# rubendhz/houdini-gsplat-renderer

Hardware: AMD Instinct MI355X
Metric: frames/sec at 1920x1080 + achieved HBM GB/s (blend kernel) (higher is better)
Workload: dtype f32

## Files before the change

houdini-gsplat-renderer_amd/csrc/gsr_api.hip:

```cpp
#include <hip/hip_runtime.h>

#include <cmath>
#include <cstddef>
#include <cstdio>
#include <cstring>
#include <chrono>
#include <algorithm>
#include <new>
#include <type_traits>
#include <vector>

#include "../../include/gsplat_hip.h"
#include "gsr_device.h"
#include "k_binning.h"
#include "k_blend.h"
#include "k_cluster.h"
#include "k_colour.h"
#include "k_preprocess.h"
#ifdef GSR_HOST_TIMING
static double g_t_verdict = 0, g_acc_py = 0, g_acc_pre = 0, g_acc_launch = 0; static long g_acc_n = 0;
static double now_us() { return std::chrono::duration<double, std::micro>(std::chrono::steady_clock::now().time_since_epoch()).count(); }
#endif
#include "k_sort.h"
#include "k_wire.h"
// ... 23 lines not shown
    bool same(const SortKey& o) const
    {
        return gen == o.gen && shard_index == o.shard_index && shard_count == o.shard_count && shard_layout == o.shard_layout && flags == o.flags &&
               band_first == o.band_first && band_tile_rows == o.band_tile_rows &&
               std::memcmp(&cam, &o.cam, sizeof(gsr_camera)) == 0;
    }
};

struct FrameArgs {
    gsr_camera cam{};
    const float* depth = nullptr;
    bool depth_is_device = false;
    float* out = nullptr;
    bool out_is_device = false;
    int aov = 0;
    float* aov_out = nullptr;
    gsr_background bg{};
};

struct FrameJob {
    FrameArgs args;
    bool open = false;
    GsrFrame f{};
    uint32_t n = 0;
    int local_tiles = 0, band_rows = 0, n_super = 0;
    size_t out_px = 0;
    float* target = nullptr;
    int format = 0;
    const float* d_depth = nullptr;
    bool timing = false, timing_all = false, use_map = false;
    bool speculative = false;
    int bn_items = 4;
    uint32_t bn_grid = 0;
    uint32_t k1_grid = 0;
    bool local_sort = false;
    bool sort_failed = false;
    bool redo = false;
    bool ranges_folded = false;
    bool deferred = false;
    bool lazy = false;
    bool cull = false;
    bool direct = false;
    uint32_t ticket = 0;
    int phase = 0;
    bool dcull = false;
    int dpar = 0;
    bool sort_fresh = false;
    bool dblind = false;
    bool dstat = false;
    bool blend_guess_plain = false;
    float2* aov_target = nullptr;
    GsrBgArgs bg{};
};

struct FrameSlot {
    hipStream_t own = nullptr;
    hipStream_t stream = nullptr;
    hipEvent_t ev_done = nullptr;
    hipEvent_t ev_user = nullptr;
    hipEvent_t ev_band[GSR_HOST_BANDS_MAX] = {nullptr, nullptr, nullptr, nullptr, nullptr, nullptr, nullptr, nullptr};
    int bands = 0;
    int band_row[GSR_HOST_BANDS_MAX + 1] = {0, 0, 0, 0, 0, 0, 0, 0, 0};
    hipEvent_t ev_pairs = nullptr;
    GsrRecord* rec = nullptr;
    uint32_t *keyA = nullptr, *keyB = nullptr;
    uint32_t* blk_cnt = nullptr;
    uint2 *valA = nullptr, *valB = nullptr;
    uint32_t* d_n = nullptr;
    float* zwin = nullptr;
    StageBuf depth_stage;
    float* dpyr = nullptr;
    size_t dpyr_cap = 0;
    uint32_t* dactive = nullptr;
    int dpar = 0;
    bool dpyr_built = false;
    bool sorted_dculled = false;
    uint32_t* hist = nullptr;
    size_t hist_cap = 0;
    uint32_t* totals = nullptr;
    uint2* pvA = nullptr;
    size_t pair_cap = 0;
    int32_t *sstart = nullptr, *send = nullptr;
    uint4* tile_work = nullptr;
    size_t tile_cap = 0;
    uint4* tile_work_a = nullptr;
    float* tbuf = nullptr;
    size_t tbuf_cap = 0;
    float* hpyr2 = nullptr;
    uint32_t* slab = nullptr;
    bool slab_dirty = false;
    int32_t* redo = nullptr;
    int32_t* order = nullptr;
    size_t order_cap = 0;
    bool order_valid = false;
    int order_age = 0;
    int order_sig[6] = {0, 0, 0, 0, 0, 0}, order_per_xcd = 0;
    uint32_t* st_scan = nullptr;
    GsrTilePartial* partial = nullptr;
    uint32_t* sup_work = nullptr;
    int sup_par = 0;
    float* hpyr = nullptr;
    float* hpyr_next = nullptr;
    float* hraw = nullptr;
    float* hstat = nullptr;
    bool hstat_valid = false;
    uint32_t* dbg_viol = nullptr;
    int hpyr_re = 0;
    uint32_t* cseg = nullptr;
    uint32_t* ccnt = nullptr;
    uint32_t* d_counts = nullptr;
    uint32_t* bkt_key = nullptr;
    uint2* bkt_val = nullptr;
    uint32_t* bkt_cnt = nullptr;
    GsrSlotHints hints;
    GsrLocalSortPolicy local_pol;
    unsigned long long* h_end = nullptr;
    unsigned long long* h_rows = nullptr;
    unsigned long long* h_rows_dev = nullptr;
    uint32_t rows_ticket = 0;
    int rows_tiles_y = 0;
    unsigned long long* h_end_dev = nullptr;
    bool horizon_valid = false;
    int horizon_sig[7] = {0, 0, 0, 0, 0, 0, 0};
    gsr_camera horizon_cam{};
    bool sorted_culled = false;
    unsigned long long* lazy_ctr = nullptr;
    uint32_t* colour_evals = nullptr;
    bool last_lazy = false;
    StageBuf fb;
    StageBuf aovb;
    float* fb32 = nullptr;
    size_t fb32_cap = 0;
    StageBuf bgb;
    unsigned long long* counters = nullptr;
    unsigned long long* h_total = nullptr;
    unsigned long long* h_total_dev = nullptr;
    uint32_t ticket = 0;
    unsigned long long* h_counters = nullptr;
    unsigned long long* d_frame = nullptr;
    bool sort_valid = false;
    SortKey sort_key{};
    uint32_t key_min = 0;
    FrameJob job;
    int last_tiles_x = 0, last_local_ty = 0, last_supers = 0;
    uint32_t last_cc_groups = 0, last_cc_per = 0;
    uint32_t last_pairs = 0;
    int super_tile = 0, stiles_x = 0, stiles_y = 0;
    uint64_t frame_id = 0;
    hipEvent_t ev[GSR_STAGE_EVENTS];
    bool ev_pending = false;
    bool ev_all = false;
    bool ev_ok = false;
};

struct gsr_context {
    int device = 0;
    hipStream_t own_stream = nullptr;
    hipStream_t stream = nullptr;

    uint32_t n = 0, cap = 0;
    bool has_sh = false;
    float origin[3] = {0, 0, 0};
    uint64_t geo_gen = 0;
    bool has_geometry = false;
    float4* geoA = nullptr;
    uint4* geoB = nullptr;
    uint4* col = nullptr;
    uint4* colrow = nullptr;
    int col_chunks = 0;
    float4* geoA2 = nullptr;
    uint4 *geoB2 = nullptr, *col2 = nullptr, *colrow2 = nullptr;
    float4 *clusA2 = nullptr, *clusB2 = nullptr;
    uint32_t* perm = nullptr;
    std::vector<int32_t> h_perm;
    float4 *clusA = nullptr, *clusB = nullptr;
    uint32_t nclus = 0;
    uint32_t* prefix = nullptr;
    uint32_t* prefix_all = nullptr;
    uint32_t* prefix_none = nullptr;
    bool prefix_valid = false;
    bool uploading = false;
    uint32_t up_total = 0, up_filled = 0;
    bool bbox_ok = false;
    double bb_lo[3] = {0, 0, 0}, bb_hi[3] = {0, 0, 0};

    FrameSlot slot[GSR_MAX_SLOTS];
    uint32_t* pos_order = nullptr;
    size_t pos_cap = 0;
    bool pos_valid = false;
    uint64_t pos_gen = 0;
    float pos_cam[3] = {0, 0, 0}, last_cam[3] = {0, 0, 0};
    uint32_t pos_kmin = 0, pos_kmax = 0;
    bool last_cam_set = false;
    uint32_t* blk_pre = nullptr;
    size_t blk_pre_cap = 0;
    int opt_order_keep = 32;
    int opt_fuse_order = 1;
    int opt_mid_sort = 1;
    int opt_host_bands = 4;
    hipStream_t copy_stream = nullptr;
    int opt_k1_scatter = 1;
    int opt_scatter_direct = 1;
    int opt_bn_items = 0;
    int nslots = 1;

    int32_t* tile_map = nullptr;
    size_t map_cap = 0;
    int map_w = 0, map_h = 0, map_si = -1, map_sc = 0, map_rpb = -1, map_first = -1, map_shift = -1, map_grid = 0;

    int shard_index = 0, shard_count = 1, shard_layout = 0;
    int band_first = 0, band_tile_rows = -1;
    int opt_row_work = 0;
    int target_format = GSR_TARGET_RGBA32F;
    int opt_swizzle = 2, opt_timing = 1, opt_sort_cache = 1, opt_super = 0, opt_flags = 0, opt_deferred = 0, opt_lazy = 1, opt_cull = 1, opt_timing_every = 1;
    int opt_cluster = 1, opt_morton = 1, opt_local_sort = 1;
    int opt_slab = 1;
    int slab_frac = 40, slab_min = 4096, slab_max = 8192;
    bool classic_once = false;

    gsr_stats st{};
    uint64_t frame_no = 0;
    size_t pair_want = 0;
    int64_t lazy_base = 0;
    uint32_t* lazy_hint = nullptr;
    bool lazy_pays = false;
    GsrCullPolicy cull_pol;
    GsrSlabPolicy slab_pol;
    bool prefix_cheaper = false;
    bool depth_active = false;
    bool order_pays = false;
    unsigned long long* wire_zbuf = nullptr;
    float* wire_out = nullptr;
    uint32_t* wire_inv = nullptr;
    uint64_t wire_inv_gen = 0;
    size_t wire_cap = 0;
    char* stage = nullptr;
    size_t stage_cap = 0;
    char* stage_raw = nullptr;
    size_t stage_raw_cap = 0;
    uint32_t *up_kA = nullptr, *up_kB = nullptr, *up_vA = nullptr, *up_vB = nullptr;
    size_t up_sort_cap = 0;
    float* up_part = nullptr;
    hipEvent_t up_ev[4] = {nullptr, nullptr, nullptr, nullptr};
    double up_t_begin = 0.0, up_h2d_ms = 0.0, up_quant_ms = 0.0;
    bool vis_on = false;
    GsrVisRule vis{};
    float* alpha0 = nullptr;
    uint32_t* vis_mask = nullptr;
    unsigned long long* vis_counters = nullptr;
    unsigned long long* vis_h_counters = nullptr;
    int64_t vis_hidden = 0;
    float* alpha0_2 = nullptr;
    uint32_t* rm_h_total = nullptr;
    int64_t rm_calls = 0, rm_last = 0;
    double rm_ms[4] = {0.0, 0.0, 0.0, 0.0};
    int64_t add_calls = 0, add_last = 0, add_grows = 0;
    double add_ms[4] = {0.0, 0.0, 0.0, 0.0};
    int64_t rd_calls = 0, rd_last = 0;
    double rd_ms[4] = {0.0, 0.0, 0.0, 0.0};
};

static inline uint32_t div_up(uint32_t a, uint32_t b) { return (a + b - 1) / b; }

#ifdef GSR_KPROF
extern "C" int gsr_debug_kprof_blocks(unsigned int* out8192) {
    hipDeviceSynchronize();
    return hipMemcpyFromSymbol(out8192, HIP_SYMBOL(g_kprof_blk), sizeof(g_kprof_blk)) == hipSuccess ? 0 : -1;
}
extern "C" int gsr_debug_kprof(unsigned long long* out128) {
    hipDeviceSynchronize();
    return hipMemcpyFromSymbol(out128, HIP_SYMBOL(g_kprof), sizeof(g_kprof)) == hipSuccess ? 0 : -1;
}
#endif
#ifdef SW_PROFILE
extern "C" int gsr_debug_sw_profile(unsigned long long* out8) {
    hipDeviceSynchronize();
    hipMemcpyFromSymbol(out8, HIP_SYMBOL(g_sw_prof), 64);
    return 0;
}
// ... 50 lines not shown
    ok = ok && hipEventCreateWithFlags(&sl.ev_pairs, hipEventDisableTiming) == hipSuccess;
    ok = ok && hipMalloc(reinterpret_cast<void**>(&sl.counters), 8 * sizeof(unsigned long long)) == hipSuccess;
    ok = ok && hipMalloc(reinterpret_cast<void**>(&sl.d_n), sizeof(uint32_t)) == hipSuccess;
    ok = ok && hipMemset(sl.d_n, 0, sizeof(uint32_t)) == hipSuccess;
    ok = ok && hipMalloc(reinterpret_cast<void**>(&sl.totals), 512 * sizeof(uint32_t)) == hipSuccess;
    ok = ok && hipMalloc(reinterpret_cast<void**>(&sl.lazy_ctr), 2 * sizeof(unsigned long long)) == hipSuccess;
    ok = ok && hipMemset(sl.lazy_ctr, 0, 2 * sizeof(unsigned long long)) == hipSuccess;
    ok = ok && hipMalloc(reinterpret_cast<void**>(&sl.colour_evals), 256 * sizeof(uint32_t)) == hipSuccess;
    ok = ok && hipMemset(sl.colour_evals, 0, 256 * sizeof(uint32_t)) == hipSuccess;
    ok = ok && hipMalloc(reinterpret_cast<void**>(&sl.hpyr), GSR_PYR_FLOATS * sizeof(float)) == hipSuccess;
    ok = ok && hipMalloc(reinterpret_cast<void**>(&sl.hpyr_next), GSR_PYR_FLOATS * sizeof(float)) == hipSuccess;
    ok = ok && hipMalloc(reinterpret_cast<void**>(&sl.hraw), (size_t)GSR_MAX_TILES_SIDE * GSR_MAX_TILES_SIDE * sizeof(float)) == hipSuccess;
    ok = ok && hipMalloc(reinterpret_cast<void**>(&sl.hstat), (size_t)GSR_MAX_TILES_SIDE * GSR_MAX_TILES_SIDE * sizeof(float)) == hipSuccess;
    ok = ok && hipMalloc(reinterpret_cast<void**>(&sl.hpyr2), GSR_PYR_FLOATS * sizeof(float)) == hipSuccess;
    ok = ok && hipMalloc(reinterpret_cast<void**>(&sl.slab), (GSR_SLAB_BINS + 8) * sizeof(uint32_t)) == hipSuccess;
    ok = ok && hipMemset(sl.slab, 0, (GSR_SLAB_BINS + 8) * sizeof(uint32_t)) == hipSuccess;
    ok = ok && hipMalloc(reinterpret_cast<void**>(&sl.ccnt), CC_MAX_GROUPS * sizeof(uint32_t)) == hipSuccess;
    ok = ok && hipMalloc(reinterpret_cast<void**>(&sl.bkt_key), (size_t)BK_BUCKETS * BK_CAP * sizeof(uint32_t)) == hipSuccess;
    ok = ok && hipMalloc(reinterpret_cast<void**>(&sl.bkt_val), (size_t)BK_BUCKETS * BK_CAP * sizeof(uint2)) == hipSuccess;
    ok = ok && hipMalloc(reinterpret_cast<void**>(&sl.bkt_cnt), (size_t)BK_BUCKETS * BK_STRIDE * sizeof(uint32_t)) == hipSuccess;
    ok = ok && hipMemset(sl.bkt_cnt, 0, (size_t)BK_BUCKETS * BK_STRIDE * sizeof(uint32_t)) == hipSuccess;
    ok = ok && hipMalloc(reinterpret_cast<void**>(&sl.d_counts), 4 * sizeof(uint32_t)) == hipSuccess;
    ok = ok && hipMemset(sl.d_counts, 0, 4 * sizeof(uint32_t)) == hipSuccess;
    ok = ok && hipHostMalloc(reinterpret_cast<void**>(&sl.h_end), sizeof(unsigned long long), hipHostMallocMapped | hipHostMallocCoherent) == hipSuccess;
    if (ok) sl.h_end[0] = 0ull;
    ok = ok && hipHostGetDevicePointer(reinterpret_cast<void**>(&sl.h_end_dev), sl.h_end, 0) == hipSuccess;
    ok = ok && hipMalloc(reinterpret_cast<void**>(&sl.st_scan), 512 * sizeof(uint32_t)) == hipSuccess;
    ok = ok && hipMemset(sl.st_scan, 0, 512 * sizeof(uint32_t)) == hipSuccess;
    ok = ok && hipMalloc(reinterpret_cast<void**>(&sl.partial), (size_t)(GSR_MAX_TILES_SIDE / 8) * (GSR_MAX_TILES_SIDE / 8) * sizeof(GsrTilePartial)) == hipSuccess;
    ok = ok && hipMalloc(reinterpret_cast<void**>(&sl.sup_work), 512 * sizeof(uint32_t)) == hipSuccess;
    ok = ok && hipMemset(sl.sup_work, 0, 512 * sizeof(uint32_t)) == hipSuccess;
    ok = ok && hipHostMalloc(reinterpret_cast<void**>(&sl.h_total), 4 * sizeof(unsigned long long), hipHostMallocMapped | hipHostMallocCoherent) == hipSuccess;
    if (ok) { sl.h_total[0] = 0ull; sl.h_total[1] = 0ull; sl.h_total[2] = 0ull; sl.h_total[3] = 0ull; }
    ok = ok && hipHostGetDevicePointer(reinterpret_cast<void**>(&sl.h_total_dev), sl.h_total, 0) == hipSuccess;
    ok = ok && hipHostMalloc(reinterpret_cast<void**>(&sl.h_counters), 8 * sizeof(unsigned long long), 0) == hipSuccess;
    if (ok) for (int j = 0; j < 8; ++j) sl.h_counters[j] = 0;
    ok = ok && hipMalloc(reinterpret_cast<void**>(&sl.d_frame), 8 * sizeof(unsigned long long)) == hipSuccess;
    ok = ok && hipMemset(sl.d_frame, 0, 8 * sizeof(unsigned long long)) == hipSuccess;
    ok = ok && hipMemset(sl.counters, 0, 8 * sizeof(unsigned long long)) == hipSuccess;
    if (ok) {
        for (int k = 0; k < GSR_STAGE_EVENTS; ++k) sl.ev[k] = nullptr;
        sl.ev_ok = true;
        for (int k = 0; k < GSR_STAGE_EVENTS && ok; ++k) ok = hipEventCreate(&sl.ev[k]) == hipSuccess;
    }
    return ok;
}

static void slot_free_splat_arrays(FrameSlot& sl)
{
    dev_free(sl.rec); dev_free(sl.keyA); dev_free(sl.keyB); dev_free(sl.valA); dev_free(sl.valB); dev_free(sl.blk_cnt);
    dev_free(sl.zwin); dev_free(sl.cseg);
    sl.sort_valid = false;
}

struct SlotSplatArrays {
    GsrRecord* rec = nullptr;
    uint32_t *keyA = nullptr, *keyB = nullptr, *blk_cnt = nullptr, *cseg = nullptr;
    uint2 *valA = nullptr, *valB = nullptr;
    float* zwin = nullptr;
    void release() { dev_free(rec); dev_free(keyA); dev_free(keyB); dev_free(valA); dev_free(valB); dev_free(blk_cnt); dev_free(zwin); dev_free(cseg); }
};
static int alloc_splat_arrays(SlotSplatArrays& a, size_t cap)
{
    int rc = GSR_OK;
    if ((rc = dev_alloc(&a.rec, cap)) || (rc = dev_alloc(&a.keyA, cap + 256)) || (rc = dev_alloc(&a.keyB, cap + 256)) ||
        (rc = dev_alloc(&a.valA, cap + 256)) || (rc = dev_alloc(&a.valB, cap + 256)) ||
        (rc = dev_alloc(&a.zwin, cap)) || (rc = dev_alloc(&a.blk_cnt, cap / 256 + 16)) ||
        (rc = dev_alloc(&a.cseg, cap / GSR_CLUSTER + (size_t)CC_THREADS * 64 + 16)))
        a.release();
    return rc;
}
static void slot_take_splat_arrays(FrameSlot& sl, SlotSplatArrays& a)
{
    slot_free_splat_arrays(sl);
    sl.rec = a.rec; sl.keyA = a.keyA; sl.keyB = a.keyB; sl.valA = a.valA; sl.valB = a.valB; sl.blk_cnt = a.blk_cnt; sl.zwin = a.zwin; sl.cseg = a.cseg;
    a = SlotSplatArrays{};
}

static void slot_destroy(FrameSlot& sl)
{
    slot_free_splat_arrays(sl);
    dev_free(sl.hist); dev_free(sl.totals);
    dev_free(sl.pvA);
    dev_free(sl.sstart); dev_free(sl.send); dev_free(sl.tile_work); dev_free(sl.order); dev_free(sl.sup_work); sl.fb.release(); dev_free(sl.fb32); sl.aovb.release(); sl.bgb.release();
    dev_free(sl.hpyr); dev_free(sl.hpyr_next); dev_free(sl.hraw); dev_free(sl.hstat); dev_free(sl.hpyr2); dev_free(sl.slab); dev_free(sl.tile_work_a); dev_free(sl.tbuf); dev_free(sl.ccnt); dev_free(sl.bkt_key); dev_free(sl.bkt_val); dev_free(sl.bkt_cnt); dev_free(sl.d_counts); dev_free(sl.st_scan); dev_free(sl.partial);
    if (sl.h_end) (void)hipHostFree(sl.h_end); if (sl.h_rows) (void)hipHostFree(sl.h_rows); sl.depth_stage.release(); dev_free(sl.dpyr); dev_free(sl.dactive);
    dev_free(sl.redo); dev_free(sl.lazy_ctr); dev_free(sl.colour_evals);
    dev_free(sl.counters); dev_free(sl.d_n);
    if (sl.h_total) (void)hipHostFree(sl.h_total);
    if (sl.h_counters) (void)hipHostFree(sl.h_counters);
    dev_free(sl.d_frame);
    if (sl.ev_ok)
        for (int k = 0; k < GSR_STAGE_EVENTS; ++k)
            if (sl.ev[k]) (void)hipEventDestroy(sl.ev[k]);
    if (sl.ev_done) (void)hipEventDestroy(sl.ev_done);
    if (sl.ev_user) (void)hipEventDestroy(sl.ev_user);
    for (int k = 0; k < GSR_HOST_BANDS_MAX; ++k) if (sl.ev_band[k]) (void)hipEventDestroy(sl.ev_band[k]);
    if (sl.ev_pairs) (void)hipEventDestroy(sl.ev_pairs);
    if (sl.own) (void)hipStreamDestroy(sl.own);
}

extern "C" int gsr_create(int device, gsr_context** out)
{
    if (!out) return set_err(GSR_E_INVALID, "gsr_create: out is NULL");
    *out = nullptr;
    int ndev = gsr_device_count();
    if (ndev <= 0) return set_err(GSR_E_NO_DEVICE, "gsr_create: no HIP device visible");
    if (device < 0 || device >= ndev) return set_err(GSR_E_NO_DEVICE, "gsr_create: device %d out of range (0..%d)", device, ndev - 1);
    HIP_TRY(hipSetDevice(device));
    gsr_context* c = new (std::nothrow) gsr_context();
    if (!c) return set_err(GSR_E_OOM, "gsr_create: host allocation failed");
    c->device = device;
    if (const char* e = std::getenv("GSR_ORDER_KEEP")) c->opt_order_keep = std::atoi(e);
    if (const char* e = std::getenv("GSR_SCATTER_DIRECT")) c->opt_scatter_direct = std::atoi(e);
    if (const char* e = std::getenv("GSR_K1_SCATTER")) c->opt_k1_scatter = std::atoi(e);
    if (const char* e = std::getenv("GSR_HOST_BANDS")) c->opt_host_bands = std::min(std::max(std::atoi(e), 1), GSR_HOST_BANDS_MAX);
    if (const char* e = std::getenv("GSR_MID_SORT")) c->opt_mid_sort = std::atoi(e);
    if (const char* e = std::getenv("GSR_FUSE_ORDER")) c->opt_fuse_order = std::atoi(e);
    if (const char* e = std::getenv("GSR_SLAB_FRAC")) { const int v = std::atoi(e); if (v >= 1 && v <= 255) c->slab_frac = v; }
    if (const char* e = std::getenv("GSR_SLAB_MIN")) { const int v = std::atoi(e); if (v >= 1) c->slab_min = v; }
    if (const char* e = std::getenv("GSR_SLAB_MAX")) { const int v = std::atoi(e); if (v >= 1) c->slab_max = v; }
    if (const char* e = std::getenv("GSR_BN_ITEMS")) { const int v = std::atoi(e); if (v == 1 || v == 2 || v == 4) c->opt_bn_items = v; }
    hipError_t e = hipStreamCreateWithFlags(&c->own_stream, hipStreamNonBlocking);
    if (e != hipSuccess) { delete c; return set_err(GSR_E_HIP, "hipStreamCreate failed: %s", hipGetErrorString(e)); }
    c->stream = c->own_stream;
    bool ok = true;
    for (int k = 0; k < GSR_MAX_SLOTS && ok; ++k) ok = slot_init(c->slot[k]);
    if (!ok) {
        gsr_destroy(c);
        return set_err(GSR_E_HIP, "gsr_create: allocating frame slots (streams/events/mailboxes) failed");
    }
    if (hipMalloc(reinterpret_cast<void**>(&c->prefix), 256 * 4) != hipSuccess ||
        hipMalloc(reinterpret_cast<void**>(&c->prefix_all), 256 * 4) != hipSuccess ||
        hipMalloc(reinterpret_cast<void**>(&c->prefix_none), 256 * 4) != hipSuccess ||
        hipMemset(c->prefix, 0xff, 256 * 4) != hipSuccess || hipMemset(c->prefix_all, 0xff, 256 * 4) != hipSuccess ||
        hipMemset(c->prefix_none, 0, 256 * 4) != hipSuccess ||
        hipMalloc(reinterpret_cast<void**>(&c->lazy_hint), 4) != hipSuccess || hipMemset(c->lazy_hint, 0, 4) != hipSuccess) {
        gsr_destroy(c);
        return set_err(GSR_E_HIP, "gsr_create: allocating the colour-prefix tables failed");
    }
    c->st.record_bytes = (int32_t)sizeof(GsrRecord);
    c->st.pair_bytes = 8;
    *out = c;
    return GSR_OK;
}

static void vis_drop_mask(gsr_context* c)
{
    dev_free(c->vis_mask);
    if (c->vis.n_volumes == 0) { c->vis_on = false; c->vis_hidden = 0; }
}

static void free_geometry(gsr_context* c)
{
    dev_free(c->geoA); dev_free(c->geoB); dev_free(c->col); dev_free(c->colrow);
    dev_free(c->perm); dev_free(c->clusA); dev_free(c->clusB); c->nclus = 0; c->h_perm.clear();
    dev_free(c->geoA2); dev_free(c->geoB2); dev_free(c->col2); dev_free(c->colrow2); dev_free(c->clusA2); dev_free(c->clusB2);
    dev_free(c->alpha0);
    dev_free(c->alpha0_2);
    vis_drop_mask(c);
    for (int k = 0; k < GSR_MAX_SLOTS; ++k) slot_free_splat_arrays(c->slot[k]);
    c->cap = 0; c->n = 0;
}

extern "C" void gsr_destroy(gsr_context* c)
{
    if (!c) return;
    (void)hipSetDevice(c->device);
    (void)sync_all(c);
    gsr_internal_comm_release(c);
    free_geometry(c);
    for (int k = 0; k < GSR_MAX_SLOTS; ++k) slot_destroy(c->slot[k]);
    dev_free(c->tile_map);
    dev_free(c->wire_zbuf); dev_free(c->wire_out); dev_free(c->wire_inv); dev_free(c->stage); dev_free(c->stage_raw);
    dev_free(c->up_kA); dev_free(c->up_kB); dev_free(c->up_vA); dev_free(c->up_vB); dev_free(c->up_part);
    for (int k = 0; k < 4; ++k) if (c->up_ev[k]) (void)hipEventDestroy(c->up_ev[k]);
    dev_free(c->prefix); dev_free(c->prefix_all); dev_free(c->prefix_none); dev_free(c->lazy_hint);
    dev_free(c->pos_order); dev_free(c->blk_pre); dev_free(c->vis_counters);
    if (c->vis_h_counters) (void)hipHostFree(c->vis_h_counters);
    if (c->rm_h_total) (void)hipHostFree(c->rm_h_total);
    if (c->own_stream) (void)hipStreamDestroy(c->own_stream);
    if (c->copy_stream) (void)hipStreamDestroy(c->copy_stream);
    delete c;
}

extern "C" int gsr_set_stream(gsr_context* c, void* s)
{
    if (!c) return set_err(GSR_E_INVALID, "gsr_set_stream: ctx is NULL");
    if (gsr_internal_comm_set_user_stream(c, s, c->own_stream)) return GSR_OK;
    HIP_TRY(hipSetDevice(c->device));
    int rc = sync_all(c);
    if (rc) return rc;
    c->stream = s ? reinterpret_cast<hipStream_t>(s) : c->own_stream;
    for (int k = 0; k < GSR_MAX_SLOTS; ++k) c->slot[k].stream = c->slot[k].own;
    return GSR_OK;
}

extern "C" int gsr_set_option(gsr_context* c, int option, int value)
{
    if (!c) return set_err(GSR_E_INVALID, "gsr_set_option: ctx is NULL");
    switch (option) {
// ... 849 lines not shown
    c->st.ms_tile_sort = ms[3] + ms[4];
    c->st.ms_blend = ms[5];
    float tot = 0.0f;
    (void)hipEventElapsedTime(&tot, e[0], e[6]);
    c->st.ms_total = tot;
    c->st.blend_ms_total += ms[5];
    c->st.blend_launches += 1;
    c->st.frame_ms_total += tot;
    c->st.stage_ms_total[0] += ms[0];
    c->st.stage_ms_total[1] += ms[1];
    c->st.stage_ms_total[2] += ms[2];
    c->st.stage_ms_total[3] += ms[3] + ms[4];
    c->st.stage_ms_total[4] += ms[5];
    c->st.stage_frames += 1;
}

static inline int mark(FrameSlot& sl, int k)
{
    const FrameJob& j = sl.job;
    if (j.timing && (j.timing_all || k >= 5)) HIP_TRY(hipEventRecord(sl.ev[k], sl.stream));
    return GSR_OK;
}

static GsrRangeArgs range_args(gsr_context* c, FrameSlot& sl)
{
    const FrameJob& j = sl.job;
    GsrRangeArgs a;
    a.totals = sl.totals; a.n_super = j.n_super; a.sstart = sl.sstart; a.send = sl.send; a.host_total = sl.h_total_dev;
    a.ticket = j.ticket; a.max_pairs = (unsigned long long)GSR_MAX_PAIRS; a.redo_count = reinterpret_cast<uint32_t*>(sl.lazy_ctr);
    a.lazy_hint = c->lazy_hint; a.n_sorted = sl.d_n; a.k1_counts = sl.d_counts; a.sorted_keys = sl.keyA;
    a.depth_active = j.dcull ? sl.dactive + j.dpar : (const uint32_t*)nullptr;
    return a;
}

static inline void tile_sig(const GsrFrame& f, int* sig )
{
    const int now[6] = {f.width, f.height, f.shard_rpb > 0 ? f.shard_first : f.shard_index, f.shard_count, f.shard_rpb, f.super_shift};
    std::memcpy(sig, now, sizeof now);
}

static inline int32_t list_cap(const FrameSlot& sl) { return (int32_t)std::min<size_t>(sl.pair_cap, (size_t)0x7fffffff); }

static GsrSumArgs sum_args(const FrameJob& j)
{
    GsrSumArgs g;
    g.n_tiles = j.local_tiles; g.tiles_x = j.f.tiles_x; g.tiles_y = j.f.tiles_y; g.shard = gsr_frame_shard(j.f, 0);
    g.super_shift = j.f.super_shift; g.stiles_x = j.f.stiles_x; g.n_super = j.n_super;
    return g;
}

static GsrHorizonArgs horizon_args(const gsr_context* c, const FrameSlot& sl)
{
    const GsrFrame& f = sl.job.f;
    GsrHorizonArgs hz{};
    hz.list_cap = list_cap(sl); hz.lists = sl.pvA; hz.geoA = c->geoA; hz.idx_mask = f.idx_mask;
    for (int l = 0; l < GSR_PYR_LEVELS; ++l) hz.pyr_off[l] = f.pyr_off[l];
    hz.cam[0] = f.cam[0]; hz.cam[1] = f.cam[1]; hz.cam[2] = f.cam[2];
    return hz;
}

static int queue_blend(gsr_context* c, FrameSlot& sl, bool with_depth, bool guarded)
{
    const FrameJob& j = sl.job;
    const GsrFrame& f = j.f;
    hipStream_t s = sl.stream;
    if (j.local_tiles <= 0) return GSR_OK;
    if (!j.direct) HIP_TRY(hipStreamWaitEvent(s, sl.ev_user, 0));
    GsrBlendArgs a;
    a.guard = guarded ? sl.dactive + j.dpar : (const uint32_t*)nullptr; a.guard_want = 0u;
    {
        const bool persp = f.pr[8] == 0.0f && f.pr[9] == 0.0f && f.pr[12] == 0.0f && f.pr[13] == 0.0f && f.pr[14] == -1.0f && f.pr[15] == 0.0f;
        a.near_alpha = persp ? 0.5f * (1.0f - f.pr[10]) : 0.0f;
        a.near_scale = persp ? 1.12f : 0.0f;
    }
    a.tile_cov = (with_depth && j.dcull && !j.dblind) ? sl.dpyr + 4 * sl.dpyr_cap : (const float*)nullptr;
    a.idx_mask = f.idx_mask; a.zq0 = f.zq0; a.zqs = f.zqs;
    a.tile_dmax = (with_depth && j.dcull && !j.dblind && f.idx_mask != 0xffffffffu) ? sl.dpyr + (size_t)(2 * j.dpar) * sl.dpyr_cap + f.pyr_off[0] : (const float*)nullptr;
    a.width = f.width; a.height = f.height; a.tiles_x = f.tiles_x; a.local_tiles = j.local_tiles;
    a.shard = gsr_frame_shard(f, 0); a.band_rows = j.band_rows;
    a.super_shift = f.super_shift; a.rect_shift = f.rect_shift; a.stiles_x = f.stiles_x; a.use_map = j.use_map ? 1 : 0; a.flags = f.flags;
    a.list_cap = list_cap(sl);
    a.sup_work = (a.use_map && c->opt_swizzle >= 2 && sl.sup_work) ? sl.sup_work + 256 * sl.sup_par : nullptr;
    a.slab = j.phase; a.tbuf = sl.tbuf; a.tile_work_a = sl.tile_work_a;
    uint4* const tw = j.phase == 1 ? sl.tile_work_a : sl.tile_work;
    int sig[6];
    tile_sig(f, sig);
    const bool ordered = a.use_map && c->opt_swizzle >= 2 && sl.order_valid && std::memcmp(sig, sl.order_sig, sizeof sig) == 0;
    const int32_t* tmap = ordered ? sl.order : c->tile_map;
    const unsigned grid = ordered ? (unsigned)(8 * sl.order_per_xcd) : a.use_map ? (unsigned)c->map_grid : (unsigned)j.local_tiles;
    GsrLazyArgs lz;
    lz.f = f; lz.colrow = c->colrow;
    lz.redo = j.lazy ? sl.redo : nullptr;
    lz.redo_count = reinterpret_cast<uint32_t*>(sl.lazy_ctr);
    const bool over = j.bg.kind != 0;
    a.out_format = j.format; a.out_packed = (j.format != GSR_TARGET_RGBA32F || over) ? (void*)j.target : nullptr;
    float4* tgt = reinterpret_cast<float4*>((j.format != GSR_TARGET_RGBA32F || over) ? sl.fb32 : j.target);
    auto launch = [&](auto kernel, unsigned g, const int32_t* map, uint4* work, auto... tail) {
        hipLaunchKernelGGL(kernel, dim3(g), dim3(256), 0, s, a, map, sl.pvA, sl.sstart, sl.send, sl.rec, tgt, work, sl.zwin, j.d_depth, lz, tail...);
    };
    auto launch_verb = [&](auto plain, auto aov, auto bg, unsigned g, const int32_t* map, uint4* work) {
        if (j.aov_target) launch(aov, g, map, work, j.aov_target);
        else if (over) launch(bg, g, map, work, j.bg);
        else launch(plain, g, map, work);
    };
    int nb = 1;
    if (!j.args.out_is_device && j.phase != 1 && c->opt_host_bands > 1 && c->shard_count == 1 && c->band_tile_rows < 0 && f.local_tiles_y >= 4 * c->opt_host_bands) nb = c->opt_host_bands;
    if (nb > 1 && !c->copy_stream && hipStreamCreateWithFlags(&c->copy_stream, hipStreamNonBlocking) != hipSuccess) { c->copy_stream = nullptr; nb = 1; (void)hipGetLastError(); }
    for (int b = 0; b < nb && nb > 1; ++b)
        if (!sl.ev_band[b] && hipEventCreateWithFlags(&sl.ev_band[b], hipEventDisableTiming) != hipSuccess) { sl.ev_band[b] = nullptr; nb = 1; (void)hipGetLastError(); }
    sl.bands = nb;
    for (int b = 0; b < nb; ++b) {
        a.row_lo = nb > 1 ? (int)((int64_t)f.local_tiles_y * b / nb) : 0;
        a.row_hi = nb > 1 ? (int)((int64_t)f.local_tiles_y * (b + 1) / nb) : 0x7fffffff;
        sl.band_row[b] = a.row_lo; sl.band_row[b + 1] = nb > 1 ? a.row_hi : f.local_tiles_y;
        if (with_depth) launch_verb(k_blend<true>, k_blend_aov<true>, k_blend_over<true>, grid, tmap, tw);
        else launch_verb(k_blend<false>, k_blend_aov<false>, k_blend_over<false>, grid, tmap, tw);
        if (j.lazy && with_depth) launch_verb(k_blend_lazy<true>, k_blend_aov_lazy<true>, k_blend_over_lazy<true>, (unsigned)j.local_tiles, c->tile_map, sl.tile_work);
        else if (j.lazy) launch_verb(k_blend_lazy<false>, k_blend_aov_lazy<false>, k_blend_over_lazy<false>, (unsigned)j.local_tiles, c->tile_map, sl.tile_work);
        if (nb > 1) HIP_TRY(hipEventRecord(sl.ev_band[b], s));
    }
    HIP_TRY(hipGetLastError());
    return GSR_OK;
}

static int queue_back_end(gsr_context* c, FrameSlot& sl)
{
    const FrameJob& j = sl.job;
    const GsrFrame& f = j.f;
    hipStream_t s = sl.stream;
    int rc;
    if ((rc = mark(sl, 3))) return rc;
    if (j.n > 0) {
        const uint32_t nblk = div_up(j.n, (uint32_t)BN_THREADS * (uint32_t)j.bn_items);
        const size_t lds = (size_t)4 * j.bn_items * j.n_super * (8 + 4);
        const GsrShard shd = gsr_frame_shard(f, f.rect_shift);
        const GsrRangeArgs ra = j.ranges_folded ? range_args(c, sl) : GsrRangeArgs{};
        const uint32_t bn_extra = (uint32_t)BN_SPLIT_TILES * (uint32_t)std::max(f.stiles_y - 1, 0);
        const uint32_t grid = std::min(nblk, j.bn_grid) + bn_extra + (j.ranges_folded ? 1u : 0u);
#define GSR_PLACE(I) hipLaunchKernelGGL((f.idx_mask != 0xffffffffu ? k_bin_place<I, true> : k_bin_place<I, false>), dim3(grid), dim3(BN_THREADS), lds, s, sl.valA, sl.d_n,          \
                                        f.super_shift - f.rect_shift, shd, f.stiles_x, j.n_super, sl.hist, sl.sstart, nblk, (uint32_t)sl.pair_cap, sl.pvA, ra,   \
                                        f.idx_mask != 0xffffffffu ? sl.zwin : (const float*)nullptr, f.zq0, f.zqs)
        if (j.bn_items == 1) GSR_PLACE(1); else if (j.bn_items == 2) GSR_PLACE(2); else GSR_PLACE(4);
#undef GSR_PLACE
        HIP_TRY(hipGetLastError());
    }
    if ((rc = mark(sl, 4))) return rc;
    if (j.lazy && j.n > 0) {
        const bool predict = c->prefix_valid && !(f.flags & GSR_FLAG_LAZY_NO_PREFIX);
        hipLaunchKernelGGL(k_colour_prefix, dim3((unsigned)(j.n_super * CL_BLOCKS_PER_LIST)), dim3(CL_THREADS), 0, s, f, sl.pvA,
                           sl.sstart, sl.send, (f.flags & GSR_FLAG_LAZY_NO_PREFIX) ? c->prefix_none : (predict ? c->prefix : c->prefix_all),
                           (int)list_cap(sl), c->colrow, sl.rec, sl.colour_evals);
        HIP_TRY(hipGetLastError());
    }
    if ((rc = mark(sl, 5))) return rc;
    sl.job.blend_guess_plain = j.d_depth != nullptr && j.dcull && !c->depth_active && !j.deferred && j.f.idx_mask == 0xffffffffu && !j.aov_target && j.bg.kind == 0;
    if ((rc = queue_blend(c, sl, j.d_depth != nullptr && !sl.job.blend_guess_plain, sl.job.blend_guess_plain))) return rc;
    return mark(sl, 6);
}

static int queue_frame_end(gsr_context* c, FrameSlot& sl)
{
    const FrameJob& j = sl.job;
    hipStream_t s = sl.stream;
    const GsrSumArgs g = sum_args(j);
    GsrHorizonArgs hz{};
    hz.list_cap = list_cap(sl);
    if (c->opt_cull && c->opt_cull != 3 && j.n > 0 && !j.deferred && (c->opt_cull >= 2 || j.cull || j.phase == 2 || (c->cull_pol.vis_unculled >= 300000u && c->cull_pol.holdoff <= 2))) {
        hz = horizon_args(c, sl);
        hz.raw = sl.hraw; hz.pyr_in = sl.hpyr; hz.pyr_out = sl.hpyr_next; hz.dilate = j.f.cull_dilate; hz.culled = j.cull ? 1 : 0;
        hz.host_end = j.cull ? sl.h_end_dev : nullptr; hz.ticket = j.ticket;
        hz.stat = sl.hstat;
        hz.stat_in_use = (j.cull && j.dcull && j.dstat) ? 1 : 0;
        hz.depth_culled = (j.dcull && !j.dblind) ? 1 : 0;
        static const bool dbgv = std::getenv("GSR_DEBUG_VIOL") != nullptr;
        if (dbgv) {
            if (!sl.dbg_viol && hipMalloc(reinterpret_cast<void**>(&sl.dbg_viol), 80 * 4) != hipSuccess) sl.dbg_viol = nullptr;
            if (sl.dbg_viol) (void)hipMemsetAsync(sl.dbg_viol, 0, 80 * 4, s);
            hz.dbg = sl.dbg_viol;
        }
    }
    if (j.phase == 2) { hz.slab = 2; hz.tile_work_a = sl.tile_work_a; }
    const int nblocks8 = ((j.f.tiles_x + 7) >> 3) * ((j.f.tiles_y + 7) >> 3);
    hipLaunchKernelGGL(k_tile_pass, dim3((unsigned)nblocks8), dim3(64), 0, s, sl.tile_work, g, sl.sstart, sl.send, hz, sl.partial, sl.st_scan);
    uint32_t* const prefix_arg = (j.f.sh_order > 0 && c->opt_lazy) ? c->prefix : (uint32_t*)nullptr;
    const uint32_t* const redo_arg = j.lazy ? reinterpret_cast<const uint32_t*>(sl.lazy_ctr) : (const uint32_t*)nullptr;
    uint32_t* const work_next = sl.sup_work ? sl.sup_work + 256 * (sl.sup_par ^ 1) : (uint32_t*)nullptr;
    sl.horizon_valid = hz.raw != nullptr;
    sl.hstat_valid = hz.raw != nullptr;
    int osig[6];
    tile_sig(j.f, osig);
    const bool order_due = c->opt_swizzle >= 3 || (c->opt_swizzle == 2 && c->order_pays);
    const bool order_kept = !order_due && c->opt_swizzle == 2 && c->opt_order_keep > 0 && sl.order_valid && sl.order_age < c->opt_order_keep &&
                            std::memcmp(osig, sl.order_sig, sizeof osig) == 0;
    const bool order_refresh = !order_due && !order_kept && c->opt_swizzle == 2 && c->opt_order_keep > 0 && c->n >= 1000000u;
    if (order_kept) sl.order_age += 1; else sl.order_valid = false;
    const bool order_now = j.use_map && (order_due || order_refresh) && j.local_tiles > 0 && j.n_super <= 256 && sl.sup_work;
    const int per_xcd = 2 * ((j.n_super + 15) / 16) << (2 * j.f.super_shift);
    if (order_now && (size_t)8 * per_xcd > sl.order_cap) {
        const int rc = regrow(s, sl.order, sl.order_cap, (size_t)8 * per_xcd, (size_t)8 * per_xcd);
        if (rc) return rc;
    }
    const bool fused_order = order_now && c->opt_fuse_order != 0;
    if (sl.horizon_valid) sl.hpyr_re = std::min(c->cull_pol.dilate, GSR_DILATE_EXACT_MAX);
    if (fused_order) {
        const GsrOrderArgs oa{sl.tile_work, j.f.tiles_y, sl.sup_work + 256 * sl.sup_par, per_xcd, sl.order};
        const int ndil = sl.horizon_valid ? nblocks8 : 0;
        hipLaunchKernelGGL(k_frame_end_order, dim3(9u + (unsigned)((ndil + TO_THREADS / 64 - 1) / (TO_THREADS / 64))), dim3(TO_THREADS), 0, s, sl.partial, nblocks8, ndil, g, sl.counters, sl.d_n, sl.d_frame,
                           prefix_arg, redo_arg, sl.colour_evals, sl.lazy_ctr + 1, sl.sstart, sl.send, c->lazy_hint, work_next, hz, sl.st_scan, sl.hpyr_re, oa);
        HIP_TRY(hipGetLastError());
    } else if (sl.horizon_valid) {
        hipLaunchKernelGGL(k_frame_end, dim3((unsigned)nblocks8 + 1u), dim3(SW_THREADS), 0, s, sl.partial, nblocks8, g, sl.counters, sl.d_n, sl.d_frame,
                           prefix_arg, redo_arg, sl.colour_evals, sl.lazy_ctr + 1, sl.sstart, sl.send, c->lazy_hint, work_next, hz, sl.st_scan, sl.hpyr_re);
        HIP_TRY(hipGetLastError());
    } else {
        hipLaunchKernelGGL(k_sum_work, dim3(1), dim3(SW_THREADS), 0, s, sl.partial, nblocks8, g, sl.counters, sl.d_n, sl.d_frame,
                           prefix_arg, redo_arg, sl.colour_evals, sl.lazy_ctr + 1, sl.sstart, sl.send, c->lazy_hint, work_next, hz, sl.st_scan);
        HIP_TRY(hipGetLastError());
    }
    if (sl.horizon_valid) {
        std::swap(sl.hpyr, sl.hpyr_next);
        tile_sig(j.f, sl.horizon_sig);
        sl.horizon_sig[6] = (int)c->geo_gen;
        sl.horizon_cam = j.args.cam;
    }
    if (order_now) {
        if (!fused_order) {
            hipLaunchKernelGGL(k_tile_order, dim3(8), dim3(TO_THREADS), 0, s, sl.tile_work, g, j.f.tiles_y, sl.sup_work + 256 * sl.sup_par,
                               per_xcd, sl.order);
            HIP_TRY(hipGetLastError());
        }
        std::memcpy(sl.order_sig, osig, sizeof osig);
        sl.order_per_xcd = per_xcd;
        sl.order_valid = true;
        sl.order_age = 0;
    }
    if (c->opt_row_work && sl.h_rows_dev) {
        hipLaunchKernelGGL(k_row_work, dim3((unsigned)((j.f.tiles_y + RW_THREADS / 64 - 1) / (RW_THREADS / 64))), dim3(RW_THREADS), 0, s, sl.tile_work,
                           j.phase == 2 ? sl.tile_work_a : (const uint4*)nullptr, g, sl.h_rows_dev, j.ticket);
        HIP_TRY(hipGetLastError());
        sl.rows_ticket = j.ticket; sl.rows_tiles_y = j.f.tiles_y;
    }
    sl.sup_par ^= 1;
    if (j.f.sh_order > 0 && c->opt_lazy) c->prefix_valid = j.phase == 0;
    sl.last_lazy = j.lazy;
    if (j.timing) { sl.ev_pending = true; sl.ev_all = j.timing_all; }
    if (!j.args.out_is_device) {
        const size_t bpp = (size_t)gsr_format_pixel_bytes(j.format);
        if (sl.bands > 1 && c->copy_stream) {
            for (int b = 0; b < sl.bands; ++b) {
                const size_t r0 = std::min<size_t>((size_t)sl.band_row[b] * GSR_TILE, (size_t)j.band_rows), r1 = std::min<size_t>((size_t)sl.band_row[b + 1] * GSR_TILE, (size_t)j.band_rows);
                if (r1 <= r0) continue;
                const size_t off = r0 * (size_t)j.f.width * bpp;
                HIP_TRY(hipStreamWaitEvent(c->copy_stream, sl.ev_band[b], 0));
                HIP_TRY(hipMemcpyAsync(reinterpret_cast<char*>(j.args.out) + off, static_cast<const char*>(sl.fb.p) + off, (r1 - r0) * (size_t)j.f.width * bpp, hipMemcpyDeviceToHost, c->copy_stream));
            }
            HIP_TRY(hipStreamSynchronize(c->copy_stream));
        } else {
            HIP_TRY(hipMemcpyAsync(j.args.out, sl.fb.p, j.out_px * bpp, hipMemcpyDeviceToHost, s));
        }
        if (j.aov_target) HIP_TRY(hipMemcpyAsync(j.args.aov_out, sl.aovb.p, j.out_px * 8, hipMemcpyDeviceToHost, s));
        HIP_TRY(hipStreamSynchronize(s));
    }
    if (!j.direct) {
        HIP_TRY(hipEventRecord(sl.ev_done, s));
        HIP_TRY(hipStreamWaitEvent(c->stream, sl.ev_done, 0));
    }
    return GSR_OK;
}

static int queue_slab_mid(gsr_context* c, FrameSlot& sl)
{
    const FrameJob& j = sl.job;
    hipStream_t s = sl.stream;
    const GsrSumArgs g = sum_args(j);
    GsrHorizonArgs hz = horizon_args(c, sl);
    hz.raw = (c->opt_cull && c->opt_cull != 3) ? sl.hraw : nullptr;
    const int nblocks8 = ((j.f.tiles_x + 7) >> 3) * ((j.f.tiles_y + 7) >> 3);
    hipLaunchKernelGGL(k_slab_mid, dim3((unsigned)nblocks8), dim3(64), 0, s, sl.tile_work_a, g, sl.sstart, sl.send, hz, sl.hpyr2,
                       sl.slab + GSR_SLAB_BINS, j.f.key_min);
    HIP_TRY(hipGetLastError());
    return GSR_OK;
}

static int frame_abort(FrameSlot& sl, int rc)
{
    sl.job.open = false;
    if (sl.stream) (void)hipStreamSynchronize(sl.stream);
    return rc;
}

static int wait_mailbox(FrameSlot& sl, volatile unsigned long long* box, uint32_t ticket, const char* what, unsigned long long* out)
{
    unsigned long long v = *box;
    if ((uint32_t)(v >> 32) != ticket) {
        const auto t0 = std::chrono::steady_clock::now();
        for (unsigned long spins = 1; (uint32_t)(v >> 32) != ticket; ++spins) {
            if ((spins & 0xffu) == 0 && std::chrono::steady_clock::now() - t0 > std::chrono::microseconds(GSR_SPIN_US)) {
                const hipError_t q = hipStreamSynchronize(sl.stream);
                if (q != hipSuccess) return set_err(GSR_E_HIP, "gsr_render: waiting for the %s: %s", what, hipGetErrorString(q));
                v = *box;
                if ((uint32_t)(v >> 32) != ticket) return set_err(GSR_E_HIP, "gsr_render: the frame finished without delivering its %s", what);
                break;
            }
            __builtin_ia32_pause();
            v = *box;
        }
    }
    *out = v;
    return GSR_OK;
}

static bool camera_jumped(const gsr_context* c, const gsr_camera& was, const gsr_camera& now)
{
    if (!c->bbox_ok) return false;
    double diag2 = 0.0;
    for (int k = 0; k < 3; ++k) diag2 += ((double)c->bb_hi[k] - c->bb_lo[k]) * ((double)c->bb_hi[k] - c->bb_lo[k]);
    if (!(diag2 > 0.0) || !std::isfinite(diag2)) return false;
// ... 198 lines not shown
    if (!c->has_geometry) return set_err(GSR_E_NO_GEOMETRY, "gsr_render: nothing uploaded");
    HIP_TRY(hipSetDevice(c->device));

    FrameSlot& sl = c->slot[c->frame_no % (uint64_t)c->nslots];
    slot = &sl;
    int rc = frame_finish(c, sl);
    if (rc) return rc;
    hipStream_t want = (c->nslots == 1) ? c->stream : sl.own;
    if (want != sl.stream) {
        HIP_TRY(hipStreamSynchronize(sl.stream));
        sl.stream = want;
    }
    if (sl.pair_cap > 0 && sl.pair_cap < c->pair_want && (rc = regrow(sl.stream, sl.pvA, sl.pair_cap, c->pair_want + 4, c->pair_want))) return rc;

    FrameJob& j = sl.job;
    j = FrameJob();
    j.args = a;
    build_frame(c, cam, &j.f);
    j.n = c->n;
    j.local_tiles = j.f.tiles_x * j.f.local_tiles_y;
    j.band_rows = ctx_band_rows(c, cam->height);
    j.out_px = (size_t)j.band_rows * cam->width;
    j.n_super = j.f.stiles_x * j.f.stiles_y;
    j.use_map = c->opt_swizzle != 0;
    return GSR_OK;
}

static void plan_frame(gsr_context* c, FrameSlot& sl, FrontEnd& fe, bool allow_cull, int phase_in)
{
    FrameJob& j = sl.job;
    const FrameArgs& a = j.args;
    const gsr_camera* cam = &a.cam;
    const GsrFrame& f = j.f;
    fe.key_now = SortKey{c->geo_gen, c->shard_index, c->shard_count, c->shard_layout, c->opt_flags, c->band_first, c->band_tile_rows, *cam};
    int sig[7] = {0, 0, 0, 0, 0, 0, (int)c->geo_gen};
    tile_sig(f, sig);
    GsrPlanIn in;
    in.phase_in = phase_in; in.allow_cull = allow_cull; in.out_is_device = a.out_is_device; in.has_depth = a.depth != nullptr;
    in.n = j.n; in.nclus = c->nclus; in.sh_order = f.sh_order; in.key_min = f.key_min; in.key_max = f.key_max;
    in.opt_deferred = c->opt_deferred; in.opt_lazy = c->opt_lazy; in.opt_cull = c->opt_cull; in.opt_slab = c->opt_slab; in.opt_cluster = c->opt_cluster;
    in.opt_sort_cache = c->opt_sort_cache; in.opt_local_sort = c->opt_local_sort; in.opt_k1_scatter = c->opt_k1_scatter;
    in.opt_scatter_direct = c->opt_scatter_direct; in.opt_mid_sort = c->opt_mid_sort; in.opt_bn_items = c->opt_bn_items;
    in.full_keys = (c->opt_flags & GSR_FLAG_FULL_KEYS) != 0; in.shard_count = c->shard_count;
    in.timing = c->opt_timing != 0 && (c->opt_timing >= 2 || c->frame_no % (uint64_t)c->opt_timing_every == 0);
    in.timing_all = c->opt_timing >= 2;
    in.opt_timing = c->opt_timing;
    in.lazy_pays = c->lazy_pays; in.prefix_cheaper = c->prefix_cheaper; in.prefix_valid = c->prefix_valid; in.bbox_ok = c->bbox_ok;
    in.horizon_match = sl.horizon_valid && std::memcmp(sig, sl.horizon_sig, sizeof sig) == 0;
    in.hpyr_re = sl.hpyr_re;
    in.sort_match = sl.sort_valid && sl.sort_key.same(fe.key_now);
    in.sorted_culled = sl.sorted_culled; in.sorted_dculled = sl.sorted_dculled;
    in.pos_match = c->pos_valid && c->pos_gen == c->geo_gen && std::memcmp(c->pos_cam, cam->cam_pos, sizeof c->pos_cam) == 0 &&
                   c->pos_kmin == f.key_min && c->pos_kmax == f.key_max;
    in.same_pos = c->last_cam_set && std::memcmp(c->last_cam, cam->cam_pos, sizeof c->last_cam) == 0;
    in.hints = sl.hints;
    fe.pos_match = in.pos_match;
    fe.p = gsr_plan_frame(in, c->cull_pol, c->slab_pol, sl.local_pol, c->classic_once, [&] { return camera_jumped(c, sl.horizon_cam, *cam); });
    const GsrFramePlan& p = fe.p;
    j.deferred = p.deferred; j.lazy = p.lazy; j.cull = p.cull; j.phase = p.phase; j.timing = p.timing; j.timing_all = p.timing_all;
    j.dcull = p.dcull; j.local_sort = p.local || p.local_phase; j.bn_items = p.bn_items; j.bn_grid = p.bn_grid; j.k1_grid = p.k1_grid;
    j.f.cull_dilate = p.cull_dilate;
    j.f.phase = p.phase;
    c->st.frames_jumped += p.jumped;
    c->st.frames_culled += p.cull;
    c->st.frames_slab += p.phase == 1;
    c->st.frames_lazy += p.lazy && j.n > 0 && phase_in == 0;
    j.ticket = ++sl.ticket ? sl.ticket : ++sl.ticket;
    if (j.timing) harvest_slot(c, sl);
}

static int stage_frame_buffers(gsr_context* c, FrameSlot& sl)
{
    FrameJob& j = sl.job;
    const FrameArgs& a = j.args;
    const gsr_camera* cam = &a.cam;
    const GsrFrame& f = j.f;
    hipStream_t s = sl.stream;
    int rc;
    j.direct = sl.stream == c->stream;
    if (!j.direct) HIP_TRY(hipEventRecord(sl.ev_user, c->stream));

    if ((size_t)j.local_tiles + 1 > sl.tile_cap || !sl.sstart) {
        HIP_TRY(hipStreamSynchronize(s));
        dev_free(sl.tile_work); dev_free(sl.tile_work_a); dev_free(sl.sstart); dev_free(sl.send); dev_free(sl.redo);
        sl.tile_cap = 0;
        if ((rc = dev_alloc(&sl.tile_work, (size_t)j.local_tiles + 1)) || (rc = dev_alloc(&sl.tile_work_a, (size_t)j.local_tiles + 1)) || (rc = dev_alloc(&sl.sstart, (size_t)65536 + 1)) ||
            (rc = dev_alloc(&sl.send, (size_t)65536 + 1)) || (rc = dev_alloc(&sl.redo, (size_t)j.local_tiles + 1))) return rc;
        sl.tile_cap = (size_t)j.local_tiles + 1;
    }
    if (j.phase == 1 && j.out_px > sl.tbuf_cap && (rc = regrow(s, sl.tbuf, sl.tbuf_cap, j.out_px, j.out_px))) return rc;
    if (j.use_map && (rc = build_tile_map(c, f))) return rc;
    j.d_depth = a.depth;
    if (a.depth && !a.depth_is_device) {
        if ((rc = sl.depth_stage.upload(s, a.depth, (size_t)cam->width * cam->height * sizeof(float)))) return rc;
        j.d_depth = static_cast<const float*>(sl.depth_stage.p);
    }
    if (a.bg.kind != 0) {
        j.bg.kind = a.bg.kind; j.bg.format = a.bg.format;
        std::memcpy(j.bg.rgba, a.bg.rgba, sizeof j.bg.rgba);
        j.bg.image = a.bg.kind == GSR_BG_IMAGE ? a.bg.image : nullptr;
        if (a.bg.kind == GSR_BG_IMAGE && !a.bg.image_is_device) {
            if ((rc = sl.bgb.upload(s, a.bg.image, (size_t)cam->width * cam->height * (size_t)gsr_format_pixel_bytes(a.bg.format)))) return rc;
            j.bg.image = sl.bgb.p;
        }
    }
    if (j.dcull) {
        frame_depth_codes(c, cam, &j.f);
        const size_t need = (size_t)f.pyr_off[GSR_PYR_LEVELS - 1] + (size_t)gsr_pyr_dim(f.tiles_x, GSR_PYR_LEVELS - 1) * gsr_pyr_dim(f.tiles_y, GSR_PYR_LEVELS - 1) + 16;
        if (need > sl.dpyr_cap || !sl.dactive) {
            if ((rc = regrow(s, sl.dpyr, sl.dpyr_cap, 5 * need, need))) return rc;
            HIP_TRY(hipMemsetAsync(sl.dpyr, 0, 5 * need * sizeof(float), s));
            if (!sl.dactive) {
                if ((rc = dev_alloc(&sl.dactive, 2))) return rc;
                HIP_TRY(hipMemsetAsync(sl.dactive, 0, 2 * sizeof(uint32_t), s));
            }
        }
        if (j.phase != 2) sl.dpar ^= 1;
        j.dpar = sl.dpar;
    }
    j.target = a.out;
    j.format = c->target_format;
    const size_t bpp = (size_t)gsr_format_pixel_bytes(j.format);
    if ((j.format != GSR_TARGET_RGBA32F || a.bg.kind != 0) && j.phase == 1 && j.out_px * 4 > sl.fb32_cap && (rc = regrow(s, sl.fb32, sl.fb32_cap, j.out_px * 4, j.out_px * 4))) return rc;
    int band[6];
    tile_sig(f, band);
    if (!a.out_is_device) {
        band[5] = j.format;
        if ((rc = sl.fb.ensure(s, j.out_px * bpp)) || (rc = sl.fb.clear_if_reshaped(s, band, j.out_px * bpp))) return rc;
        j.target = static_cast<float*>(sl.fb.p);
    }
    if (a.aov != 0 && a.aov_out != nullptr) {
        j.aov_target = reinterpret_cast<float2*>(a.aov_out);
        if (!a.out_is_device) {
            band[5] = 0;
            if ((rc = sl.aovb.ensure(s, j.out_px * sizeof(float2))) || (rc = sl.aovb.clear_if_reshaped(s, band, j.out_px * sizeof(float2)))) return rc;
            j.aov_target = static_cast<float2*>(sl.aovb.p);
        }
    }
    return GSR_OK;
}

static int queue_pos_order(gsr_context* c, FrameSlot& sl, FrontEnd& fe)
{
    if (fe.p.want_pos && !fe.pos_match) {
        c->pos_valid = false;
        if (const int rc = fe.p.ordered ? build_pos_order(c, sl, sl.job.f, fe.p.key_bits) : GSR_OK) return rc;
    }
    std::memcpy(c->last_cam, sl.job.args.cam.cam_pos, sizeof c->last_cam);
    c->last_cam_set = true;
    return GSR_OK;
}

static int queue_cull(gsr_context* c, FrameSlot& sl, FrontEnd& fe)
{
    FrameJob& j = sl.job;
    const GsrFrame& f = j.f;
    const GsrFramePlan& p = fe.p;
    hipStream_t s = sl.stream;
    if (j.n == 0) return GSR_OK;
    cluster_grid(c->nclus, &fe.rounds, &fe.ngroups);
    if ((c->opt_flags & GSR_FLAG_CULL_ROUNDS) && c->nclus > 0) {
        fe.rounds = std::max(fe.rounds, 3);
        fe.ngroups = div_up(c->nclus, (uint32_t)CC_THREADS * (uint32_t)fe.rounds);
    }
    fe.hist_shift = p.key_bits > 10 ? p.key_bits - 10 : 0;
    const float* pyr = j.phase == 2 ? sl.hpyr2 : ((j.cull && !p.ordered) ? sl.hpyr : (const float*)nullptr);
    const GsrSlabPick pk{(uint32_t)c->slab_min, (uint32_t)c->slab_max, (uint32_t)c->slab_frac, f.key_max - f.key_min};
    GsrDepthPyrArgs& dp = fe.dp;
    if (j.dcull) {
        float* const dp0 = sl.dpyr + (size_t)(2 * j.dpar) * sl.dpyr_cap;
// ... 391 lines not shown
    if (n_pixels == 0) return GSR_OK;
    HIP_TRY(hipSetDevice(c->device));
    hipLaunchKernelGGL(k_resolve_depth, dim3((unsigned)((n_pixels + 255) / 256)), dim3(256), 0, c->stream, reinterpret_cast<const float2*>(aov), n_pixels, cov_min, depth_out);
    HIP_TRY(hipGetLastError());
    return GSR_OK;
}

__attribute__((visibility("hidden"))) int gsr_internal_frame_begin(gsr_context* c, const gsr_camera* cam, const float* depth,
                                                                    int depth_is_device, float* out_dev)
{
    if (!c || !cam || !out_dev) return set_err(GSR_E_INVALID, "gsr_render: NULL argument");
    if (!target_aligned(c, out_dev)) return set_err(GSR_E_INVALID, "gsr_render: the device target is not aligned to its %d-byte pixel", gsr_format_pixel_bytes(c->target_format));
    if (c->band_tile_rows == 0) return GSR_OK;
    return frame_begin(c, FrameArgs{*cam, depth, depth_is_device != 0, out_dev, true}, nullptr, true);
}
__attribute__((visibility("hidden"))) int gsr_internal_frame_finish(gsr_context* c) { return c ? finish_open_frames(c) : GSR_OK; }
__attribute__((visibility("hidden"))) int gsr_internal_frame_check(gsr_context* c, const gsr_camera* cam, const float* depth,
                                                                    int depth_is_device, float* out_dev)
{
    FrameSlot* sl = c ? latest_slot(c) : nullptr;
    if (!sl || c->band_tile_rows == 0) return GSR_OK;
    if (!cam || !out_dev) return set_err(GSR_E_INVALID, "gsr_render: NULL argument");
    return frame_check(c, *sl, FrameArgs{*cam, depth, depth_is_device != 0, out_dev, true});
}
__attribute__((visibility("hidden"))) void* gsr_internal_stream(gsr_context* c) { return c ? (void*)c->stream : nullptr; }
__attribute__((visibility("hidden"))) int gsr_internal_device(gsr_context* c) { return c ? c->device : -1; }

static int render_wire(gsr_context* c, const gsr_camera* cam, float* rgba_out, int out_is_device, int over);
extern "C" int gsr_render_wire(gsr_context* c, const gsr_camera* cam, float* rgba_out, int out_is_device) { return render_wire(c, cam, rgba_out, out_is_device, 0); }
extern "C" int gsr_render_wire_over(gsr_context* c, const gsr_camera* cam, float* rgba_inout, int is_device) { return render_wire(c, cam, rgba_inout, is_device, 1); }
static int render_wire(gsr_context* c, const gsr_camera* cam, float* rgba_out, int out_is_device, int over)
{
    if (!c || !cam || !rgba_out) return set_err(GSR_E_INVALID, "gsr_render_wire: NULL argument");
    if (c->uploading) return set_err(GSR_E_INVALID, "gsr_render_wire: upload in progress");
    if (cam->width <= 0 || cam->height <= 0 || cam->width > GSR_MAX_DIM || cam->height > GSR_MAX_DIM)
        return set_err(GSR_E_INVALID, "gsr_render_wire: bad framebuffer size %dx%d", cam->width, cam->height);
    if (!c->has_geometry) return set_err(GSR_E_NO_GEOMETRY, "gsr_render_wire: nothing uploaded");
    if (out_is_device && !target_aligned(c, rgba_out)) return set_err(GSR_E_INVALID, "gsr_render_wire: the device target is not aligned to its %d-byte pixel", gsr_format_pixel_bytes(c->target_format));
    const size_t bpp = (size_t)gsr_format_pixel_bytes(c->target_format);
    HIP_TRY(hipSetDevice(c->device));
    int rc = sync_all(c);
    if (rc) return rc;
    hipStream_t s = c->slot[0].own;
    GsrFrame f;
    build_frame(c, cam, &f);
    const size_t npix = (size_t)cam->width * cam->height;
    if (npix > c->wire_cap) {
        dev_free(c->wire_zbuf); dev_free(c->wire_out);
        c->wire_cap = 0;
        if ((rc = dev_alloc(&c->wire_zbuf, npix)) || (rc = dev_alloc(&c->wire_out, npix * 4))) {
            dev_free(c->wire_zbuf); dev_free(c->wire_out);
            return rc;
        }
        c->wire_cap = npix;
    }
    if ((rc = ensure_inverse_perm(c))) return rc;
    const uint32_t* const inv = (c->perm && c->n > 0) ? c->wire_inv : (const uint32_t*)nullptr;
    unsigned long long* zbuf = c->wire_zbuf;
    float* target = out_is_device ? rgba_out : c->wire_out;
    hipError_t e = hipMemsetAsync(zbuf, 0xff, npix * 8, s);
    if (e == hipSuccess && over && !out_is_device) e = hipMemcpyAsync(c->wire_out, rgba_out, npix * bpp, hipMemcpyHostToDevice, s);
    if (e == hipSuccess && c->n > 0)
        hipLaunchKernelGGL(k_wire_splats, dim3(div_up(c->n, 256)), dim3(256), 0, s, c->n, f, c->geoA, c->geoB, zbuf, inv ? c->perm : (const uint32_t*)nullptr);
    if (e == hipSuccess)
        hipLaunchKernelGGL(k_wire_resolve, dim3((unsigned)((npix + 255) / 256)), dim3(256), 0, s, zbuf, npix, c->col,
                           target, c->target_format, inv, over);
    if (e == hipSuccess) e = hipGetLastError();
    if (e == hipSuccess && !out_is_device) e = hipMemcpyAsync(rgba_out, c->wire_out, npix * bpp, hipMemcpyDeviceToHost, s);
    if (e == hipSuccess) e = hipStreamSynchronize(s);
    if (e != hipSuccess) return set_err(GSR_E_HIP, "gsr_render_wire: %s", hipGetErrorString(e));
    return GSR_OK;
}

extern "C" int gsr_debug_policy(int32_t* state16, int event, long long a, long long b)
{
    if (!state16) return set_err(GSR_E_INVALID, "gsr_debug_policy: NULL state");
    gsr_policy_apply(state16, event, a, b);
    return state16[11] < 0 ? set_err(GSR_E_INVALID, "gsr_debug_policy: unknown event %d", event) : GSR_OK;
}
extern "C" int gsr_debug_frame_plan(int which, const int32_t* in, int32_t* policy16, int32_t* out)
{
    if (!in || !out || (which == 0 && !policy16)) return set_err(GSR_E_INVALID, "gsr_debug_frame_plan: NULL argument");
    return gsr_frame_plan_apply(which, in, policy16, out) ? set_err(GSR_E_INVALID, "gsr_debug_frame_plan: unknown selector %d", which) : GSR_OK;
}
extern "C" int gsr_debug_policy_state(gsr_context* c, int32_t* state16)
{
    if (!c || !state16) return set_err(GSR_E_INVALID, "gsr_debug_policy_state: NULL argument");
    const GsrCullPolicy& p = c->cull_pol;
    const int32_t v[GSR_POLICY_STATE_INTS] = {p.pays, p.weak, (int32_t)p.vis_unculled, p.holdoff, p.backoff, p.streak, p.dilate, p.opt_dilate,
                                              c->slab_pol.holdoff, c->slot[0].local_pol.fails, c->slot[0].local_pol.holdoff, 0, 0, 0, 0, 0};
    std::memcpy(state16, v, sizeof v);
    return GSR_OK;
}

extern "C" int gsr_synchronize(gsr_context* c)
{
    if (!c) return set_err(GSR_E_INVALID, "gsr_synchronize: ctx is NULL");
    HIP_TRY(hipSetDevice(c->device));
    int rc = sync_all(c);
    return rc ? rc : gsr_internal_comm_sync(c);
}

static void fetch_counters(gsr_context* c)
{
    for (int k = 0; k < GSR_MAX_SLOTS; ++k)
        if (c->slot[k].d_frame && c->slot[k].h_counters)
            (void)hipMemcpy(c->slot[k].h_counters, c->slot[k].d_frame, 8 * sizeof(unsigned long long), hipMemcpyDeviceToHost);
}

static FrameSlot* latest_slot(gsr_context* c)
{
    FrameSlot* best = nullptr;
    for (int k = 0; k < GSR_MAX_SLOTS; ++k)
        if (c->slot[k].frame_id && (!best || c->slot[k].frame_id > best->frame_id)) best = &c->slot[k];
    return best;
}

extern "C" int gsr_get_stats(gsr_context* c, gsr_stats* out)
{
    if (!c || !out) return set_err(GSR_E_INVALID, "gsr_get_stats: NULL argument");
    HIP_TRY(hipSetDevice(c->device));
    int rc = sync_all(c);
    if (rc) return rc;
    fetch_counters(c);
    FrameSlot* last = latest_slot(c);
    for (int k = 0; k < GSR_MAX_SLOTS; ++k)
        if (&c->slot[k] != last) harvest_slot(c, c->slot[k]);
    if (last) {
        harvest_slot(c, *last);
        FrameSlot& sl = *last;
        c->st.n_visible = (int64_t)(sl.h_counters[6] & 0xffffffffull);
        c->st.lazy_redo_tiles = sl.last_lazy ? (int64_t)(sl.h_counters[7] & 0xffffffffull) : 0;
        c->st.pairs_consumed = (int64_t)sl.h_counters[1];
        c->st.entries_scanned = (int64_t)sl.h_counters[3];
        c->st.pairs_total = sl.last_pairs;
        c->st.clusters_total = c->nclus;
        c->st.clusters_kept = sl.hints.surv_hint;
        c->st.policy_bits = (c->lazy_pays ? 1 : 0) | (c->order_pays ? 2 : 0) | (c->cull_pol.pays ? 4 : 0) | (c->cull_pol.weak ? 8 : 0) | (c->prefix_cheaper ? 16 : 0) | (c->depth_active ? 32 : 0);
        c->st.cull_dilate = c->cull_pol.dilate;
        c->st.cull_holdoff = c->cull_pol.holdoff;
        c->st.tiles_x = sl.last_tiles_x;
        c->st.tiles_y = sl.last_local_ty;
        c->st.super_tile = sl.super_tile;
        c->st.stiles_x = sl.stiles_x;
        c->st.stiles_y = sl.stiles_y;
        int64_t rec_tot = 0, ent_tot = 0, ev_tot = 0;
        for (int k = 0; k < GSR_MAX_SLOTS; ++k) {
            if (!c->slot[k].frame_id) continue;
            rec_tot += (int64_t)c->slot[k].h_counters[2];
            ent_tot += (int64_t)c->slot[k].h_counters[4];
            ev_tot += (int64_t)c->slot[k].h_counters[5];
        }
        c->st.blend_pairs_consumed_total = rec_tot;
        c->st.blend_entries_scanned_total = ent_tot;
        c->st.blend_wave_evals_total = ev_tot;
        {
            unsigned long long tot = 0, v = 0;
            for (int k = 0; k < GSR_MAX_SLOTS; ++k)
                if (c->slot[k].lazy_ctr && hipMemcpy(&v, c->slot[k].lazy_ctr + 1, 8, hipMemcpyDeviceToHost) == hipSuccess) tot += v;
            c->st.lazy_colours_total = (int64_t)tot - c->lazy_base;
        }
    }
    *out = c->st;
    return GSR_OK;
}

// ... 312 lines not shown
```

houdini-gsplat-renderer_amd/csrc/gsr_frame_plan.h:

```cpp
#pragma once
#include <algorithm>
#include <cstdint>
#include "gsr_mailbox.h"
#include "gsr_policy.h"

struct GsrSlotHints {
    uint32_t surv_hint = 0;
    uint32_t kept_hint = 0;
    uint32_t kept_lo = 0, kept_hi = 0;
    bool kept_culled = false;
    uint32_t slab_kept = 0;
    uint32_t slab_kept1 = 0, slab_kept2 = 0;
};

enum : uint32_t { GSR_PLAN_K1_THREADS = 256, GSR_PLAN_BN_THREADS = 256, GSR_PLAN_BK_BUCKETS = 1024, GSR_PLAN_CLUSTER = 64 };

static inline uint32_t gsr_plan_div_up(uint32_t a, uint32_t b) { return (a + b - 1) / b; }

#define GSR_PLAN_IN_FIELDS(X)                                                                                                      \
    X(int, phase_in)                                               \
    X(bool, allow_cull)                                  \
    X(bool, out_is_device)                                                                                                      \
    X(bool, has_depth)                                                                                \
    X(uint32_t, n)                                                                                         \
// ... 129 lines not shown
    GSR_BE_KEPT = 0,
    GSR_BE_QUEUED = 1,
    GSR_BE_REQUEUED = 2,
    GSR_BE_TRUNCATED = 3,
};

#define GSR_OUTCOME_IN_FIELDS(X)                                                                                                   \
    X(bool, has_splats)                                                                      \
    X(int, phase) X(bool, cull) X(bool, local_sort) X(bool, dcull) X(bool, dblind) X(bool, speculative) X(bool, deferred)       \
    X(bool, blend_guess_plain)                                                                                                  \
    X(uint32_t, key_min)                                                                                                        \
    X(uint64_t, pair_cap) X(bool, has_list_buffer)                                                                              \
    X(uint64_t, max_pairs)                                                                                                      \
    X(uint32_t, mb_pairs) X(uint32_t, mb_hints) X(uint32_t, mb_kept) X(uint32_t, mb_clusters) X(uint32_t, mb_key_lo) X(uint32_t, mb_key_hi)

#define GSR_OUTCOME_OUT_FIELDS(X)                                                                                                  \
    X(int, end)                                                                                                \
    X(int, back_end)                                                                                        \
    X(bool, grow)                                             \
    X(bool, guard_miss)          \
    X(int, local_result)                           \
    X(int, depth_active)                                      \
    X(bool, verdicts)           \
    X(bool, kept_counts)                                          \
    X(bool, slab_done)

#define GSR_PLAN_DECLARE(t, name) t name{};
struct GsrOutcomeIn { GSR_OUTCOME_IN_FIELDS(GSR_PLAN_DECLARE) };
struct GsrFrameOutcome { GSR_OUTCOME_OUT_FIELDS(GSR_PLAN_DECLARE) };
#undef GSR_PLAN_DECLARE

inline GsrFrameOutcome gsr_frame_outcome(const GsrOutcomeIn& in, GsrSlotHints& h)
{
    GsrFrameOutcome o;
    o.local_result = -1;
    o.depth_active = -1;
    if (!in.has_splats) return o;
    const bool covered = (in.mb_hints & GSR_HINT_DEPTH_COVERED) != 0u;
    if (in.local_sort && (in.mb_hints & GSR_HINT_SORT_GAVE_UP)) {
        o.end = GSR_FE_SORT_GAVE_UP;
        o.local_result = 1;
        h.kept_hint = 0; h.kept_lo = h.kept_hi = 0;
        return o;
    }
    if (in.local_sort) o.local_result = 0;
    if (in.dcull && in.dblind && in.cull && covered) {
        o.end = GSR_FE_DEPTH_APPEARED;
        o.depth_active = 1;
        return o;
    }
    if (in.dcull) o.depth_active = covered ? 1 : 0;
    o.verdicts = in.phase != 2;
    if (in.phase == 0) {
        o.kept_counts = true;
        h.surv_hint = in.mb_clusters;
        h.kept_hint = in.mb_kept;
        h.kept_culled = in.cull;
    } else if (in.phase == 1) {
        h.slab_kept = in.mb_kept; h.slab_kept1 = std::max(in.mb_kept, 1u);
    } else {
        h.slab_kept2 = std::max(in.mb_kept, 1u);
        h.kept_hint = h.slab_kept + in.mb_kept;
        o.slab_done = true;
        h.surv_hint = std::min<uint32_t>(in.mb_clusters, std::max<uint32_t>(16384u, 2u * gsr_plan_div_up(h.kept_hint, GSR_PLAN_CLUSTER)));
        h.kept_culled = true;
    }
    if (h.kept_hint > 0 && in.phase == 0) {
        h.kept_lo = in.mb_key_lo + in.key_min;
        h.kept_hi = in.mb_key_hi + in.key_min;
    } else {
        h.kept_lo = h.kept_hi = 0;
    }
    if (in.mb_pairs == GSR_MB_TOO_MANY_PAIRS || in.mb_pairs > in.max_pairs) { o.end = GSR_FE_TOO_MANY_PAIRS; return o; }
    o.grow = in.mb_pairs > in.pair_cap || !in.has_list_buffer;
    if (o.grow && in.speculative && in.phase == 2) { o.end = GSR_FE_SLAB_OVERRUN; return o; }
    if (in.deferred) o.back_end = o.grow ? GSR_BE_TRUNCATED : GSR_BE_KEPT;
    else if (!in.speculative) o.back_end = GSR_BE_QUEUED;
    else o.back_end = o.grow ? GSR_BE_REQUEUED : GSR_BE_KEPT;
    o.guard_miss = o.back_end == GSR_BE_KEPT && in.blend_guess_plain && covered;
    o.end = in.phase == 1 ? GSR_FE_PHASE_2 : GSR_FE_DONE;
    return o;
}

#define GSR_PLAN_HINT_FIELDS(X) X(uint32_t, surv_hint) X(uint32_t, kept_hint) X(uint32_t, kept_lo) X(uint32_t, kept_hi) X(bool, kept_culled) \
    X(uint32_t, slab_kept) X(uint32_t, slab_kept1) X(uint32_t, slab_kept2)
inline int gsr_frame_plan_apply(int which, const int32_t* in, int32_t* policy, int32_t* out)
{
    int k = 0, o = 0;
#define GSR_GET(t, name) v.name = (t)(uint32_t)in[k++];
#define GSR_GET_HINT(t, name) h.name = (t)(uint32_t)in[k++];
#define GSR_PUT(t, name) out[o++] = (int32_t)r.name;
#define GSR_PUT_HINT(t, name) out[o++] = (int32_t)h.name;
    if (which == 0) {
        GsrPlanIn v;
        GSR_PLAN_IN_FIELDS(GSR_GET)
        GsrSlotHints& h = v.hints;
        GSR_PLAN_HINT_FIELDS(GSR_GET_HINT)
        bool classic_once = in[k++] != 0;
        GsrCullPolicy c; GsrSlabPolicy s; GsrLocalSortPolicy l;
        c.pays = policy[0] != 0; c.weak = policy[1] != 0; c.vis_unculled = (uint32_t)policy[2]; c.holdoff = policy[3]; c.backoff = policy[4];
        c.streak = policy[5]; c.dilate = policy[6]; c.opt_dilate = policy[7]; s.holdoff = policy[8]; l.fails = policy[9]; l.holdoff = policy[10];
        const GsrFramePlan r = gsr_plan_frame(v, c, s, l, classic_once, [&] { return v.jumped; });
        GSR_PLAN_OUT_FIELDS(GSR_PUT)
        out[o++] = classic_once;
        policy[3] = c.holdoff; policy[8] = s.holdoff; policy[9] = l.fails; policy[10] = l.holdoff;
        return 0;
    }
    if (which == 1) {
        GsrOutcomeIn v;
        GSR_OUTCOME_IN_FIELDS(GSR_GET)
        GsrSlotHints h;
        GSR_PLAN_HINT_FIELDS(GSR_GET_HINT)
        const GsrFrameOutcome r = gsr_frame_outcome(v, h);
        GSR_OUTCOME_OUT_FIELDS(GSR_PUT)
        GSR_PLAN_HINT_FIELDS(GSR_PUT_HINT)
        return 0;
    }
#undef GSR_GET
#undef GSR_GET_HINT
#undef GSR_PUT
#undef GSR_PUT_HINT
    return -1;
}
```

houdini-gsplat-renderer_amd/csrc/k_blend.h:

```cpp
#pragma once
#include <type_traits>
#include "gsr_device.h"
#include "k_preprocess.h"
#include "k_cluster.h"

#ifndef BL_ROUND
#define BL_ROUND 64
#endif
#ifndef BL_WAVES_PER_EU
#define BL_WAVES_PER_EU 6
#endif
#ifndef BL_CHECK
#define BL_CHECK 4
#endif
#ifndef BL_BATCH
#define BL_BATCH 256
#endif
#ifndef BL_CHECK_AOVD
#define BL_CHECK_AOVD 2
#endif
#define BL_QCAP 2048
#define BL_PAIR_F4_MAX 6
#define GSR_T_MIN 6.103515625e-05f

#ifdef BL_PROFILE
#define BLP_MAX_WG 65536
__device__ unsigned long long g_blend_prof[BLP_MAX_WG][4][16];
#define BLP(i) { const long long now_ = clock64(); prof[i] += (unsigned long long)(now_ - tlast); tlast = now_; }
#else
#define BLP(i)
#endif

__device__ __forceinline__ uint32_t gsr_tile_weight(const uint4& w) { return w.z * 32u + w.y * 8u + (w.x >> 1); }

#ifdef GSR_DEBUG_XCC
__device__ uint32_t g_dbg_xcc[4];
#endif
struct GsrBlendArgs {
    int32_t width, height;
    int32_t tiles_x;
    int32_t local_tiles;
    GsrShard shard;
    int32_t band_rows;
    int32_t super_shift;
    int32_t rect_shift;
    int32_t stiles_x;
    int32_t use_map;
    int32_t flags;
    int32_t list_cap;
    uint32_t* sup_work;
    int32_t slab;
    float* tbuf;
    const uint4* tile_work_a;
    const uint32_t* guard;
    uint32_t guard_want;
    float near_alpha, near_scale;
    const float* tile_cov;
    uint32_t idx_mask;
    float zq0, zqs;
    const float* tile_dmax;
    int32_t row_lo, row_hi;
    int32_t out_format;
    void* out_packed;
};

#if BL_WAVES_PER_EU > 0
#define BL_OCC __attribute__((amdgpu_waves_per_eu(BL_WAVES_PER_EU)))
#else
#define BL_OCC
#endif
struct GsrLazyArgs {
    GsrFrame f;
    const uint4* colrow;
    int32_t* redo;
    uint32_t* redo_count;
};
struct GsrBgArgs {
    int32_t kind;
    int32_t format;
    float rgba[4];
    const void* image;
};
template <bool HAS_DEPTH, bool LAZY, bool AOV = false, bool OVER = false>
__device__ __forceinline__ void
gsr_blend_tile(const GsrBlendArgs& a, const int32_t* __restrict__ tile_map, const uint2* __restrict__ svals,
               const int32_t* __restrict__ sstart, const int32_t* __restrict__ send,
               const GsrRecord* __restrict__ recs, float4* __restrict__ out, uint4* __restrict__ tile_work,
               const float* __restrict__ zwin, const float* __restrict__ depth, const GsrLazyArgs& lz, float2* __restrict__ aov = nullptr,
               const GsrBgArgs* __restrict__ bg = nullptr)
{
    constexpr bool ZSTAGE = HAS_DEPTH || AOV;
    constexpr int PF4 = 5;
    __shared__ float4 slist[4][(BL_ROUND / 2) * PF4];
    __shared__ float2 szl[ZSTAGE ? 4 : 1][ZSTAGE ? BL_ROUND / 2 : 1];
    __shared__ uint32_t q[BL_QCAP];
    __shared__ __attribute__((aligned(16))) uint32_t scnt[2][4];
    __shared__ uint32_t sdone[2][4];
    __shared__ float swmax[2][4];
    __shared__ uint32_t sevals, sredo, sdmet;
    __shared__ uint32_t slastu[4];
    __shared__ uint32_t stail[32];
    __shared__ uint32_t slast[4];

    int tile;
    if (LAZY) {
        if (blockIdx.x >= *lz.redo_count) return;
        tile = lz.redo[blockIdx.x];
    } else {
        tile = a.use_map ? tile_map[blockIdx.x] : (int)blockIdx.x;
    }
#ifdef GSR_DEBUG_XCC
    if (threadIdx.x == 0) {
        uint32_t xcc;
        asm volatile("s_getreg_b32 %0, hwreg(HW_REG_XCC_ID)" : "=s"(xcc));
        xcc &= 0xfu;
        atomicAdd(&g_dbg_xcc[(xcc == (blockIdx.x & 7u)) ? 0 : 1], 1u);
        if (blockIdx.x == 0) g_dbg_xcc[2] = xcc;
    }
#endif
    if (tile < 0 || tile >= a.local_tiles) return;
    if (a.row_hi != 0x7fffffff) { const int row = tile / a.tiles_x; if (row < a.row_lo || row >= a.row_hi) return; }
    const uint32_t guard_now = (!HAS_DEPTH && a.guard) ? *a.guard : 0u;
    const int tid = threadIdx.x, lane = tid & 63, wave = tid >> 6;
#ifdef BL_PROFILE
    unsigned long long prof[10] = {0, 0, 0, 0, 0, 0, 0, 0, 0, 0};
    unsigned long long occ_lanes = 0, occ_evals = 0, occ_half = 0, occ_none = 0;
    long long tlast = clock64();
    const unsigned long long wall0 = wall_clock64();
#endif
    const int tx = tile % a.tiles_x, lty = tile / a.tiles_x;
    const int gty = gsr_shard_global_row(a.shard, lty);
    const int px = tx * GSR_TILE_PX + (wave & 1) * 8 + (lane & 7);
    const int py = gty * GSR_TILE_PX + (wave >> 1) * 8 + (lane >> 3);
    const bool pix_ok = (px < a.width) && (py < a.height);
    const gsr_v2f lx = (gsr_v2f)((float)((wave & 1) * 8 + (lane & 7))), ly = (gsr_v2f)((float)((wave >> 1) * 8 + (lane >> 3)));
    const float tcx0 = (float)(tx * GSR_TILE_PX) + 0.5f, tcy0 = (float)(gty * GSR_TILE_PX) + 0.5f;
    const float qcx = tcx0 + 3.5f + 8.0f * (float)(wave & 1), qcy = tcy0 + 3.5f + 8.0f * (float)(wave >> 1);
    if (tid == 0) { sevals = 0; sredo = 0; sdmet = 0; }
    if (tid < 4) slast[tid] = 0u;
    uint32_t my_evals = 0;
    uint32_t my_last = 0;
    const bool tile_plain = HAS_DEPTH && a.tile_cov != nullptr && !(a.flags & GSR_FLAG_NO_DEPTH_CLASS) && a.tile_cov[gty * a.tiles_x + tx] < 0.0f;
    const float dpx = (HAS_DEPTH && pix_ok && !tile_plain) ? depth[(size_t)py * a.width + px] : __builtin_inff();
    bool d_met = false;
    bool d_triv = true, d_init = !HAS_DEPTH;
    float d_wmin = __builtin_inff();

    const int st = (gty >> a.super_shift) * a.stiles_x + (tx >> a.super_shift);
    const int s = sstart[st];
    const int e_ = send[st] < a.list_cap ? send[st] : a.list_cap;
    const int n = e_ > s ? e_ - s : 0;
    if (!HAS_DEPTH && a.guard && (guard_now != 0u) != (a.guard_want != 0u)) return;

    gsr_v2f C01 = {0.0f, 0.0f};
    float C2 = 0.0f, T = 1.0f;
    float Z = 0.0f;
    bool wave_done = false;
    if (a.slab == 2) {
        const uint4 wa = a.tile_work_a[tile];
        if (wa.w & 1u) {
            if (tid == 0) tile_work[tile] = make_uint4(0u, 0u, 0u, 1u | 0x8000u | (0xffffu << 16));
            return;
        }
        if (pix_ok) {
            const size_t at = (size_t)(lty * GSR_TILE_PX + (wave >> 1) * 8 + (lane >> 3)) * a.width + (size_t)(tx * GSR_TILE_PX + (wave & 1) * 8 + (lane & 7));
            const float4 c = out[at];
            C01 = (gsr_v2f){c.x, c.y}; C2 = c.z; T = a.tbuf[at];
            if constexpr (AOV) Z = aov[at].x;
        }
        wave_done = __all(!pix_ok || T < GSR_T_MIN);
    }
    bool u_done = false;
    uint32_t my_last_u = 0;
    uint32_t es_u = 0xffu;
    bool u_all = false;
    uint32_t fetched = 0;


    int scan_pos = 0;
    uint32_t q_head = 0, q_tail = 0;
    int spar = 0;
    uint32_t zlim = 0xffffffffu;
    const bool zfilter = HAS_DEPTH && a.tile_dmax != nullptr && a.idx_mask != 0xffffffffu && !tile_plain && !(a.flags & GSR_FLAG_NO_DEPTH_CLASS);
    if (zfilter) zlim = (gsr_zq(a.tile_dmax[gty * a.tiles_x + tx], a.zq0, a.zqs) << GSR_ZQ_SHIFT) | a.idx_mask;
    uint32_t imask = HAS_DEPTH ? a.idx_mask : 0xffffffffu;
    if (HAS_DEPTH) asm volatile("" : "+s"(imask));
    const uint32_t sub_mask = (1u << a.super_shift) - 1u;
    const uint32_t tile_bits = (1u << ((tx & sub_mask) >> a.rect_shift)) | (0x10000u << ((gty & sub_mask) >> a.rect_shift));
    typedef uint32_t gsr_u4 __attribute__((ext_vector_type(4), aligned(8)));
    gsr_u4 preA = {0u, 0u, 0u, 0u}, preB = {0u, 0u, 0u, 0u};
    auto prefetch = [&]() __attribute__((always_inline)) {
        const int i = scan_pos + 4 * tid;
        if (i < n) {
            const gsr_u4* src = reinterpret_cast<const gsr_u4*>(svals + s + i);
            preA = src[0]; preB = src[1];
        }
    };
    prefetch();
    int round = 0;
    int first_hit_step = -1;
    bool saturated = false;

    auto ext_steps_of = [&](uint32_t c) __attribute__((always_inline)) -> uint32_t {
        const int cur = (scan_pos >> 10) - 1;
        if (c == 0u) return 0u;
        if (cur < 0) return 0xffu;
        const int ln = (int)__builtin_amdgcn_mbcnt_hi(~0u, __builtin_amdgcn_mbcnt_lo(~0u, 0u));
        const bool reached = ln < 32 && cur - ln >= 0 && stail[(cur - ln) & 31] >= c;
        const unsigned long long m = __ballot(reached);
        const int k = __builtin_ctzll(~m | (1ull << 63));
        const int e = cur - (k - 1) + 1;
        return (m & 1ull) == 0ull || e <= 0 || e > 0xfe ? 0xffu : (uint32_t)e;
    };
    auto init_depth = [&]() __attribute__((always_inline)) {
        d_init = true;
        u_done = __all(!pix_ok || T < GSR_T_MIN || dpx < 1.0f);
        d_triv = __all(dpx >= 1.0f) && !(a.flags & GSR_FLAG_NO_DEPTH_CLASS);
        if (a.flags & GSR_FLAG_NO_DEPTH_CLASS) {
            d_wmin = -__builtin_inff();
        } else if (!d_triv) {
            const float ninf = -__builtin_inff();
            float vmin = pix_ok ? (dpx == dpx ? dpx : ninf) : __builtin_inff();
#pragma unroll
            for (int d = 32; d > 0; d >>= 1) vmin = __builtin_fminf(vmin, __shfl_xor(vmin, d, 64));
            d_wmin = __builtin_bit_cast(float, __builtin_amdgcn_readfirstlane(__builtin_bit_cast(int, vmin)));
        }
    };
    BLP(0)
    for (;;) {
        bool scanned_any = false;
        constexpr int batch = BL_BATCH;
        while ((int)(q_tail - q_head) < batch && scan_pos < n) {
            const int rem = n - (scan_pos + 4 * tid);
            bool h0 = rem > 0 && (preA.y & tile_bits) == tile_bits, h1 = rem > 1 && (preA.w & tile_bits) == tile_bits;
            bool h2 = rem > 2 && (preB.y & tile_bits) == tile_bits, h3 = rem > 3 && (preB.w & tile_bits) == tile_bits;
// ... 137 lines not shown
                        const unsigned long long ba = __ballot(ina), bb = __ballot(inb);
                        occ_lanes += (unsigned long long)(__builtin_popcountll(ba) + __builtin_popcountll(bb));
                        occ_evals += 2ull;
                        occ_half += (unsigned long long)(((ba != 0ull) && (((ba & 0xffffffffull) == 0ull) || ((ba >> 32) == 0ull))) ? 1 : 0) +
                                    (unsigned long long)(((bb != 0ull) && (((bb & 0xffffffffull) == 0ull) || ((bb >> 32) == 0ull))) ? 1 : 0);
                        occ_none += (unsigned long long)((ba == 0ull) ? 1 : 0) + (unsigned long long)((bb == 0ull) ? 1 : 0);
                    }
#endif
                    const float wa = T * ((ina && T >= GSR_T_MIN) ? ala : 0.0f);
                    C01 = gsr_fma2((gsr_v2f)(wa), (gsr_v2f){v3.x, v3.y}, C01);
                    C2 = gsr_fma(wa, v3.z, C2);
                    if constexpr (AOV) Z = gsr_fma(wa, o.z.x, Z);
                    T = T - wa;
                    const float wb = T * ((inb && T >= GSR_T_MIN) ? alb : 0.0f);
                    C01 = gsr_fma2((gsr_v2f)(wb), (gsr_v2f){v4.x, v4.y}, C01);
                    C2 = gsr_fma(wb, v4.z, C2);
                    if constexpr (AOV) Z = gsr_fma(wb, o.z.y, Z);
                    T = T - wb;
                };
                typedef std::integral_constant<bool, false> no_depth_t;
                typedef std::integral_constant<bool, true> depth_t;
                auto blend_pair = [&](int p, gsr_v2f& C01, float& C2, float& T) __attribute__((always_inline)) { blend_ops(no_depth_t(), load_pair(no_depth_t(), p), C01, C2, T, Z); };
                auto blend_pair_d = [&](int p, gsr_v2f& C01, float& C2, float& T) __attribute__((always_inline)) { blend_ops(depth_t(), load_pair(depth_t(), p), C01, C2, T, Z); };
#ifdef BL_EXP_DOUBLE
                {
                    gsr_v2f sC01 = C01; float sC2 = C2, sT = T;
                    for (int p2 = 0; p2 < npairs; ++p2) blend_pair(p2, sC01, sC2, sT);
                    if (sT == 123.0f) { C2 += sC2 + sC01.x; }
                }
#endif
                int p = 0;
                if (!HAS_DEPTH || !dslow) {
                    constexpr int CHK = (AOV && HAS_DEPTH) ? BL_CHECK_AOVD : BL_CHECK;
                    const int nfull = npairs & ~(CHK - 1);
                    bool stop = false;
                    for (; p < nfull && !stop; p += CHK) {
#pragma unroll
                        for (int u = 0; u < CHK; ++u) blend_pair(p + u, C01, C2, T);
                        stop = __all(!pix_ok || T < GSR_T_MIN);
                    }
                    if (!stop)
                        for (; p < npairs; ++p) blend_pair(p, C01, C2, T);
                } else {
#ifndef BL_CHECK_D
#define BL_CHECK_D 1
#endif
                    const int nfull = npairs & ~(BL_CHECK_D - 1);
                    bool stop = false;
                    for (; p < nfull && !stop; p += BL_CHECK_D) {
#pragma unroll
                        for (int u = 0; u < BL_CHECK_D; ++u) blend_pair_d(p + u, C01, C2, T);
                        stop = __all(!pix_ok || T < GSR_T_MIN);
                    }
                    if (!stop)
                        for (; p < npairs; ++p) blend_pair_d(p, C01, C2, T);
                }
                my_evals += (uint32_t)(2 * p < cnt ? 2 * p : cnt);
                BLP(4)
                if (HAS_DEPTH && !u_done && __all(!pix_ok || T < GSR_T_MIN || dpx < 1.0f)) { u_done = true; my_last_u = my_last; }
                if (__all(!pix_ok || T < GSR_T_MIN)) { wave_done = true; break; }
                __builtin_amdgcn_wave_barrier();
            }
        }
        q_head += (uint32_t)take;
        const int rpar = round & 1;
        const int wv = __builtin_amdgcn_readfirstlane(wave);
        if (HAS_DEPTH && wave_done && !u_done) { u_done = true; my_last_u = my_last; }
        if (HAS_DEPTH && zfilter) {
            const bool live = pix_ok && T >= GSR_T_MIN && !wave_done;
            float vmax = live ? (dpx == dpx ? dpx : -__builtin_inff()) : -__builtin_inff();
#pragma unroll
            for (int d = 32; d > 0; d >>= 1) vmax = __builtin_fmaxf(vmax, __shfl_xor(vmax, d, 64));
            if (lane == 0) swmax[rpar][wv] = vmax;
        }
        if (lane == 0) { sdone[rpar][wv] = (wave_done ? 1u : 0u) | ((HAS_DEPTH ? u_done : wave_done) ? 2u : 0u); slast[wv] = my_last; if (HAS_DEPTH) slastu[wv] = my_last_u; }
        ++round;
        BLP(5)
        __syncthreads();
        BLP(6)
        if (!LAZY && sredo) {
            int t3 = tile;
            asm volatile("" : "+s"(t3));
            if (tid == 0 && lz.redo) lz.redo[atomicAdd(lz.redo_count, 1u)] = t3;
            return;
        }
        if (HAS_DEPTH && zfilter) {
            const float tm = __builtin_fmaxf(__builtin_fmaxf(swmax[rpar][0], swmax[rpar][1]), __builtin_fmaxf(swmax[rpar][2], swmax[rpar][3]));
            zlim = (gsr_zq(tm, a.zq0, a.zqs) << GSR_ZQ_SHIFT) | a.idx_mask;
        }
        const uint32_t dall = sdone[rpar][0] & sdone[rpar][1] & sdone[rpar][2] & sdone[rpar][3];
        if (HAS_DEPTH && !u_all && (dall & 2u)) {
            u_all = true;
            es_u = ext_steps_of(max(max(slastu[0], slastu[1]), max(slastu[2], slastu[3])));
        }
        if ((dall & 1u) != 0u) { saturated = true; break; }
    }
    if (pix_ok) {
        int t2 = tid;
        asm volatile("" : "+v"(t2));
        const int w2 = t2 >> 6, l2 = t2 & 63;
        const int brow = lty * GSR_TILE_PX + (w2 >> 1) * 8 + (l2 >> 3);
        const int bcol = tx * GSR_TILE_PX + (w2 & 1) * 8 + (l2 & 7);
        const size_t at = (size_t)brow * a.width + bcol;
        if constexpr (OVER) {
            float4 B = make_float4(bg->rgba[0], bg->rgba[1], bg->rgba[2], bg->rgba[3]);
            if (bg->kind == GSR_BGK_IMAGE) {
                const int grow = gsr_shard_global_row(a.shard, lty) * GSR_TILE_PX + (w2 >> 1) * 8 + (l2 >> 3);
                B = gsr_background_pixel(bg->image, bg->format, (size_t)grow * a.width + bcol);
            }
            const float4 S = make_float4(C01.x, C01.y, C2, 1.0f - T);
            if (a.slab == 1) { out[at] = S; a.tbuf[at] = T; }
            const float4 o = gsr_composite_over_pixel(S, B);
            if (a.out_format == GSR_FMT_RGBA32F) reinterpret_cast<float4*>(a.out_packed)[at] = o;
            else gsr_store_packed(a.out_packed, a.out_format, at, o.x, o.y, o.z, o.w);
        } else {
            if (a.out_format == GSR_FMT_RGBA32F || a.slab == 1) out[at] = make_float4(C01.x, C01.y, C2, 1.0f - T);
            if (a.out_format != GSR_FMT_RGBA32F) gsr_store_packed(a.out_packed, a.out_format, at, C01.x, C01.y, C2, 1.0f - T);
            if (a.slab == 1) a.tbuf[at] = T;
        }
        if constexpr (AOV) aov[at] = make_float2(Z, 1.0f - T);
    }
    BLP(8)
#ifdef BL_PROFILE
    if (lane == 0 && blockIdx.x < BLP_MAX_WG) {
        unsigned long long* o = g_blend_prof[blockIdx.x][wave];
#pragma unroll
        for (int i = 0; i < 9; ++i) o[i] = prof[i];
        o[9] = 1ull; o[10] = (unsigned long long)round; o[11] = wall0; o[12] = wall_clock64();
        o[13] = occ_lanes; o[14] = occ_evals; o[15] = occ_half | (occ_none << 32);
    }
#endif
    __syncthreads();
    if (lane == 0) { atomicAdd(&sevals, my_evals); if (HAS_DEPTH && d_met) sdmet = 1u; }
    __syncthreads();
    if (HAS_DEPTH && !d_init) init_depth();
    const uint32_t es_c = ext_steps_of(max(max(slast[0], slast[1]), max(slast[2], slast[3])));
    if (!HAS_DEPTH) { u_all = saturated; es_u = es_c; }
    else if (!u_all) {
        const uint32_t dl = sdone[(round - 1) & 1][0] & sdone[(round - 1) & 1][1] & sdone[(round - 1) & 1][2] & sdone[(round - 1) & 1][3];
        if (round > 0 ? (dl & 2u) != 0u : __syncthreads_and(u_done ? 1 : 0) != 0) { u_all = true; es_u = round > 0 ? ext_steps_of(max(max(slastu[0], slastu[1]), max(slastu[2], slastu[3]))) : 0u; }
    }
    if (tid == 0) {
        const int rd = scan_pos + 1024;
        const uint32_t fs = (uint32_t)(first_hit_step < 0 ? 0 : (first_hit_step > 0x1fff ? 0x1fff : first_hit_step)) | (sdmet ? 0x2000u : 0u);
        const uint4 tw = make_uint4((uint32_t)(rd < n ? rd : n), fetched, sevals, (saturated ? 1u : 0u) | (fs << 1) | (u_all ? 0x8000u : 0u) | (es_c << 16) | (es_u << 24));
        tile_work[tile] = tw;
        if (a.sup_work && gsr_tile_weight(tw)) atomicAdd(&a.sup_work[st], gsr_tile_weight(tw));
    }
}

template <bool HAS_DEPTH>
__global__ void __launch_bounds__(256) BL_OCC
k_blend(GsrBlendArgs a, const int32_t* __restrict__ tile_map, const uint2* __restrict__ svals,
        const int32_t* __restrict__ sstart, const int32_t* __restrict__ send,
        const GsrRecord* __restrict__ recs, float4* __restrict__ out, uint4* __restrict__ tile_work,
        const float* __restrict__ zwin, const float* __restrict__ depth, GsrLazyArgs lz)
{
    gsr_blend_tile<HAS_DEPTH, false>(a, tile_map, svals, sstart, send, recs, out, tile_work, zwin, depth, lz);
}
template <bool HAS_DEPTH>
__global__ void __launch_bounds__(256)
k_blend_lazy(GsrBlendArgs a, const int32_t* __restrict__ tile_map, const uint2* __restrict__ svals,
             const int32_t* __restrict__ sstart, const int32_t* __restrict__ send,
             const GsrRecord* __restrict__ recs, float4* __restrict__ out, uint4* __restrict__ tile_work,
             const float* __restrict__ zwin, const float* __restrict__ depth, GsrLazyArgs lz)
{
    gsr_blend_tile<HAS_DEPTH, true>(a, tile_map, svals, sstart, send, recs, out, tile_work, zwin, depth, lz);
}

template <bool HAS_DEPTH>
__global__ void __launch_bounds__(256) BL_OCC
k_blend_aov(GsrBlendArgs a, const int32_t* __restrict__ tile_map, const uint2* __restrict__ svals,
            const int32_t* __restrict__ sstart, const int32_t* __restrict__ send,
            const GsrRecord* __restrict__ recs, float4* __restrict__ out, uint4* __restrict__ tile_work,
            const float* __restrict__ zwin, const float* __restrict__ depth, GsrLazyArgs lz, float2* __restrict__ aov)
{
    gsr_blend_tile<HAS_DEPTH, false, true>(a, tile_map, svals, sstart, send, recs, out, tile_work, zwin, depth, lz, aov);
}
template <bool HAS_DEPTH>
__global__ void __launch_bounds__(256)
k_blend_aov_lazy(GsrBlendArgs a, const int32_t* __restrict__ tile_map, const uint2* __restrict__ svals,
                 const int32_t* __restrict__ sstart, const int32_t* __restrict__ send,
                 const GsrRecord* __restrict__ recs, float4* __restrict__ out, uint4* __restrict__ tile_work,
                 const float* __restrict__ zwin, const float* __restrict__ depth, GsrLazyArgs lz, float2* __restrict__ aov)
{
    gsr_blend_tile<HAS_DEPTH, true, true>(a, tile_map, svals, sstart, send, recs, out, tile_work, zwin, depth, lz, aov);
}

template <bool HAS_DEPTH>
__global__ void __launch_bounds__(256) BL_OCC
k_blend_over(GsrBlendArgs a, const int32_t* __restrict__ tile_map, const uint2* __restrict__ svals,
             const int32_t* __restrict__ sstart, const int32_t* __restrict__ send,
             const GsrRecord* __restrict__ recs, float4* __restrict__ out, uint4* __restrict__ tile_work,
             const float* __restrict__ zwin, const float* __restrict__ depth, GsrLazyArgs lz, GsrBgArgs bg)
{
    gsr_blend_tile<HAS_DEPTH, false, false, true>(a, tile_map, svals, sstart, send, recs, out, tile_work, zwin, depth, lz, nullptr, &bg);
}
template <bool HAS_DEPTH>
__global__ void __launch_bounds__(256)
k_blend_over_lazy(GsrBlendArgs a, const int32_t* __restrict__ tile_map, const uint2* __restrict__ svals,
                  const int32_t* __restrict__ sstart, const int32_t* __restrict__ send,
                  const GsrRecord* __restrict__ recs, float4* __restrict__ out, uint4* __restrict__ tile_work,
                  const float* __restrict__ zwin, const float* __restrict__ depth, GsrLazyArgs lz, GsrBgArgs bg)
{
    gsr_blend_tile<HAS_DEPTH, true, false, true>(a, tile_map, svals, sstart, send, recs, out, tile_work, zwin, depth, lz, nullptr, &bg);
}

#ifdef SW_PROFILE
__device__ unsigned long long g_sw_prof[8];
#define SWP(i) { if (threadIdx.x == 0) g_sw_prof[i] = clock64(); }
#else
#define SWP(i)
#endif
#define SW_THREADS 256
#ifndef SW_HEADROOM_SHIFT
#define SW_HEADROOM_SHIFT 2
#endif
#ifndef SW_HEADROOM_ADD
#define SW_HEADROOM_ADD 1024u
#endif
struct GsrSumArgs {
    int32_t n_tiles, tiles_x, tiles_y , super_shift, stiles_x, n_super;
    GsrShard shard;
};
struct GsrHorizonArgs {
    float* raw;
    const float* pyr_in;
    float* pyr_out;
    int32_t pyr_off[GSR_PYR_LEVELS];
    int32_t culled;
    int32_t dilate;
    const uint2* lists;
    int32_t list_cap;
    const float4* geoA;
    float cam[3];
    unsigned long long* host_end;
    uint32_t ticket;
    int32_t slab;
    const uint4* tile_work_a;
    float* stat;
    int32_t stat_in_use;
// ... 256 lines not shown
        const uint32_t order_pays = ((unsigned long long)s_wmax * 3072ull > wsum && wsum > 60000000ull) ? GSR_HINT_ORDER_PAYS : 0u;
        if (lazy_hint) *lazy_hint = ((prefix && (unsigned long long)s_est * 10ull < (unsigned long long)nvis * 4ull &&
                                      s_unsat * 64u <= (uint32_t)g.n_tiles) ? GSR_HINT_LAZY_PAYS : 0u) | order_pays |
                                    ((prefix && (unsigned long long)s_est * 3ull < (unsigned long long)nvis * 2ull) ? GSR_HINT_PREFIX_CHEAPER : 0u) |
                                    ((hz.culled || ((unsigned long long)s_nfin * 10ull >= (unsigned long long)s_nused * 3ull && s_nused > 0u)) ? GSR_HINT_CULL_PAYS : 0u);
        const unsigned long long t2 = old2 + s_sum[1], t4 = old4 + s_sum[0], t5 = old5 + s_sum[2];
        counters[1] = s_sum[1]; counters[2] = t2; counters[3] = s_sum[0]; counters[4] = t4; counters[5] = t5;
        if (colour_evals) *colour_total = old_ct + s_cev;
        summary[0] = 0ull; summary[1] = s_sum[1]; summary[2] = t2; summary[3] = s_sum[0]; summary[4] = t4; summary[5] = t5;
        summary[6] = (unsigned long long)nvis;
        summary[7] = (unsigned long long)nredo;
    }
    SWP(5)
}
__global__ void __launch_bounds__(SW_THREADS)
k_sum_work(const GsrTilePartial* __restrict__ partial, int nblocks, GsrSumArgs g, unsigned long long* __restrict__ counters,
           const uint32_t* __restrict__ n_visible, unsigned long long* __restrict__ summary, uint32_t* __restrict__ prefix,
           const uint32_t* __restrict__ redo_count, uint32_t* __restrict__ colour_evals, unsigned long long* __restrict__ colour_total,
           const int32_t* __restrict__ sstart, const int32_t* __restrict__ send, uint32_t* __restrict__ lazy_hint,
           uint32_t* __restrict__ sup_work_next, GsrHorizonArgs hz, uint32_t* __restrict__ st_scan)
{
    gsr_sum_work(partial, nblocks, g, counters, n_visible, summary, prefix, redo_count, colour_evals, colour_total, sstart, send, lazy_hint,
                 sup_work_next, hz, st_scan);
}

__device__ __forceinline__ void
gsr_horizon_dilate(const float* __restrict__ raw, int tiles_x, int tiles_y, int r, const GsrHorizonArgs& hz, float* __restrict__ pyr, const int b,
                   const int lane )
{
    const int lx = (lane & 1) | ((lane >> 1) & 2) | ((lane >> 2) & 4), ly = ((lane >> 1) & 1) | ((lane >> 2) & 2) | ((lane >> 3) & 4);
    const int nbx = (tiles_x + 7) >> 3;
    const int by = b / nbx, bx = b - by * nbx;
    const int tx = bx * 8 + lx, ty = by * 8 + ly;
    const bool inside = tx < tiles_x && ty < tiles_y;
    float v = 0.0f;
    if (inside) {
        const int x0 = max(tx - r, 0), x1 = min(tx + r, tiles_x - 1), y0 = max(ty - r, 0), y1 = min(ty + r, tiles_y - 1);
        bool allc = true;
        for (int y = y0; y <= y1; ++y)
            for (int x = x0; x <= x1; ++x) {
                const float rv = raw[y * tiles_x + x];
                v = __builtin_fmaxf(v, __builtin_fabsf(rv));
                allc = allc && (__float_as_uint(rv) >> 31) == 0u;
            }
        pyr[hz.pyr_off[0] + ty * tiles_x + tx] = v;
        if (hz.stat) hz.stat[ty * tiles_x + tx] = allc ? 1.0f : 0.0f;
    }
    v = __builtin_fmaxf(v, __shfl_xor(v, 1, 64)); v = __builtin_fmaxf(v, __shfl_xor(v, 2, 64));
    if ((lane & 3) == 0 && inside) pyr[hz.pyr_off[1] + (ty >> 1) * gsr_pyr_dim(tiles_x, 1) + (tx >> 1)] = v;
    v = __builtin_fmaxf(v, __shfl_xor(v, 4, 64)); v = __builtin_fmaxf(v, __shfl_xor(v, 8, 64));
    if ((lane & 15) == 0 && inside) pyr[hz.pyr_off[2] + (ty >> 2) * gsr_pyr_dim(tiles_x, 2) + (tx >> 2)] = v;
    v = __builtin_fmaxf(v, __shfl_xor(v, 16, 64)); v = __builtin_fmaxf(v, __shfl_xor(v, 32, 64));
    if (lane == 0) {
        pyr[hz.pyr_off[3] + by * nbx + bx] = v;
        atomicMax(reinterpret_cast<uint32_t*>(pyr) + hz.pyr_off[4] + (by >> 1) * gsr_pyr_dim(tiles_x, 4) + (bx >> 1), __float_as_uint(v));
        atomicMax(reinterpret_cast<uint32_t*>(pyr) + hz.pyr_off[5] + (by >> 2) * gsr_pyr_dim(tiles_x, 5) + (bx >> 2), __float_as_uint(v));
    }
}
__global__ void __launch_bounds__(64)
k_horizon_dilate(const float* __restrict__ raw, int tiles_x, int tiles_y, int r, GsrHorizonArgs hz, float* __restrict__ pyr)
{
    gsr_horizon_dilate(raw, tiles_x, tiles_y, r, hz, pyr, (int)blockIdx.x, (int)threadIdx.x);
}

__global__ void __launch_bounds__(SW_THREADS)
k_frame_end(const GsrTilePartial* __restrict__ partial, int nblocks, GsrSumArgs g, unsigned long long* __restrict__ counters,
            const uint32_t* __restrict__ n_visible, unsigned long long* __restrict__ summary, uint32_t* __restrict__ prefix,
            const uint32_t* __restrict__ redo_count, uint32_t* __restrict__ colour_evals, unsigned long long* __restrict__ colour_total,
            const int32_t* __restrict__ sstart, const int32_t* __restrict__ send, uint32_t* __restrict__ lazy_hint,
            uint32_t* __restrict__ sup_work_next, GsrHorizonArgs hz, uint32_t* __restrict__ st_scan, int dilate_r)
{
    if ((int)blockIdx.x == nblocks) {
        gsr_sum_work(partial, nblocks, g, counters, n_visible, summary, prefix, redo_count, colour_evals, colour_total, sstart, send, lazy_hint,
                     sup_work_next, hz, st_scan);
        return;
    }
    if (threadIdx.x >= 64) return;
    gsr_horizon_dilate(hz.raw, g.tiles_x, g.tiles_y, dilate_r, hz, hz.pyr_out, (int)blockIdx.x, (int)threadIdx.x);
}

#define TO_THREADS 1024
#define TO_LEVELS 128
__device__ __forceinline__ void
gsr_tile_order(const uint4* __restrict__ tile_work, const GsrSumArgs& g, int tiles_y, const uint32_t* __restrict__ sup_work, int cap,
               int32_t* __restrict__ order, const int xcd)
{
    __shared__ uint32_t s_sup[256];
    __shared__ uint32_t s_own[64];
    __shared__ uint32_t s_hist[TO_LEVELS];
    __shared__ uint32_t s_nown, s_wmax;
    const int tid = threadIdx.x, lane = tid & 63, wave = tid >> 6;
    if (tid < 256) s_sup[tid] = tid < g.n_super ? sup_work[tid] : 0u;
    if (tid < TO_LEVELS) s_hist[tid] = 0u;
    if (tid == 0) { s_nown = 0u; s_wmax = 0u; }
    __syncthreads();
    if (tid < 256) {
        bool mine_here = false;
        if (tid < g.n_super) {
            const uint32_t mine = s_sup[tid];
            uint32_t r = 0;
            for (int u = 0; u < g.n_super; ++u) {
                const uint32_t o = s_sup[u];
                r += (o > mine || (o == mine && u < tid)) ? 1u : 0u;
            }
            const uint32_t m = r & 15u;
            mine_here = (int)(m < 8u ? m : 15u - m) == xcd;
        }
        if (mine_here) s_own[atomicAdd(&s_nown, 1u)] = (uint32_t)tid;
    }
    __syncthreads();
    const int shift2 = 2 * g.super_shift, emask = (1 << g.super_shift) - 1;
    const int items = (int)s_nown << shift2;
    auto tile_of = [&](int it, uint32_t& w) -> int {
        const int st = (int)s_own[it >> shift2], j = it & ((1 << shift2) - 1);
        const int sy = st / g.stiles_x, sx = st - sy * g.stiles_x;
        const int tx = (sx << g.super_shift) + (j & emask), gty = (sy << g.super_shift) + (j >> g.super_shift);
        w = 0u;
        if (tx >= g.tiles_x || gty >= tiles_y || !gsr_shard_owns(g.shard, gty)) return -1;
        const int lty = gsr_shard_local_row(g.shard, gty);
        const int i = lty * g.tiles_x + tx;
        if (i >= g.n_tiles) return -1;
        w = gsr_tile_weight(tile_work[i]);
        return i;
    };
    constexpr int TO_CACHE = 5;
    int ci[TO_CACHE];
    uint32_t cw[TO_CACHE];
#pragma unroll
    for (int k = 0; k < TO_CACHE; ++k) { const int it = tid + k * TO_THREADS; ci[k] = -1; cw[k] = 0u; if (it < items) ci[k] = tile_of(it, cw[k]); }
    {
        uint32_t wmax = 0;
#pragma unroll
        for (int k = 0; k < TO_CACHE; ++k) wmax = cw[k] > wmax ? cw[k] : wmax;
        for (int it = tid + TO_CACHE * TO_THREADS; it < items; it += TO_THREADS) { uint32_t w; (void)tile_of(it, w); wmax = w > wmax ? w : wmax; }
#pragma unroll
        for (int d = 32; d > 0; d >>= 1) { const uint32_t o = __shfl_xor(wmax, d, 64); wmax = o > wmax ? o : wmax; }
        if (lane == 0 && wmax) atomicMax(&s_wmax, wmax);
    }
    __syncthreads();
    const float scale = s_wmax ? (float)(TO_LEVELS - 2) / (float)s_wmax : 0.0f;
    auto level_of = [&](uint32_t w) { const int l = w ? (TO_LEVELS - 2) - (int)((float)w * scale) : TO_LEVELS - 1; return l < 0 ? 0 : l; };
#pragma unroll
    for (int k = 0; k < TO_CACHE; ++k) if (ci[k] >= 0) atomicAdd(&s_hist[level_of(cw[k])], 1u);
    for (int it = tid + TO_CACHE * TO_THREADS; it < items; it += TO_THREADS) {
        uint32_t w;
        if (tile_of(it, w) >= 0) atomicAdd(&s_hist[level_of(w)], 1u);
    }
    __syncthreads();
    if (wave == 0) {
        const uint32_t a0 = s_hist[2 * lane], a1 = s_hist[2 * lane + 1];
        uint32_t x = a0 + a1;
#pragma unroll
        for (int d = 1; d < 64; d <<= 1) { const uint32_t y = __shfl_up(x, d, 64); if (lane >= d) x += y; }
        const uint32_t ex = x - (a0 + a1);
        s_hist[2 * lane] = ex; s_hist[2 * lane + 1] = ex + a0;
        if (lane == 63) s_nown = x;
    }
    __syncthreads();
#pragma unroll
    for (int k = 0; k < TO_CACHE; ++k)
        if (ci[k] >= 0) {
            const uint32_t pos = atomicAdd(&s_hist[level_of(cw[k])], 1u);
            if ((int)pos < cap) order[8 * (int)pos + xcd] = ci[k];
        }
    for (int it = tid + TO_CACHE * TO_THREADS; it < items; it += TO_THREADS) {
        uint32_t w;
        const int i = tile_of(it, w);
        if (i >= 0) {
            const uint32_t pos = atomicAdd(&s_hist[level_of(w)], 1u);
            if ((int)pos < cap) order[8 * (int)pos + xcd] = i;
        }
    }
    for (int p = (int)s_nown + tid; p < cap; p += TO_THREADS) order[8 * p + xcd] = -1;
}
__global__ void __launch_bounds__(TO_THREADS)
k_tile_order(const uint4* __restrict__ tile_work, GsrSumArgs g, int tiles_y, const uint32_t* __restrict__ sup_work, int cap,
             int32_t* __restrict__ order)
{
    gsr_tile_order(tile_work, g, tiles_y, sup_work, cap, order, (int)blockIdx.x);
}

struct GsrOrderArgs { const uint4* tile_work; int32_t tiles_y; const uint32_t* sup_work; int32_t cap; int32_t* order; };
__global__ void __launch_bounds__(TO_THREADS)
k_frame_end_order(const GsrTilePartial* __restrict__ partial, int nblocks, int ndilate , GsrSumArgs g,
                  unsigned long long* __restrict__ counters, const uint32_t* __restrict__ n_visible, unsigned long long* __restrict__ summary,
                  uint32_t* __restrict__ prefix, const uint32_t* __restrict__ redo_count, uint32_t* __restrict__ colour_evals,
                  unsigned long long* __restrict__ colour_total, const int32_t* __restrict__ sstart, const int32_t* __restrict__ send,
                  uint32_t* __restrict__ lazy_hint, uint32_t* __restrict__ sup_work_next, GsrHorizonArgs hz, uint32_t* __restrict__ st_scan, int dilate_r,
                  GsrOrderArgs oa)
{
    const int b = (int)blockIdx.x;
    if (b < 8) {
        gsr_tile_order(oa.tile_work, g, oa.tiles_y, oa.sup_work, oa.cap, oa.order, b);
        return;
    }
    if (b == 8) {
        if (threadIdx.x >= SW_THREADS) return;
        gsr_sum_work(partial, nblocks, g, counters, n_visible, summary, prefix, redo_count, colour_evals, colour_total, sstart, send, lazy_hint,
                     sup_work_next, hz, st_scan);
        return;
    }
    static_assert(TO_THREADS % 64 == 0 && SW_THREADS % 64 == 0, "early exits are by whole wavefronts");
    const int blk = (b - 9) * (TO_THREADS / 64) + (int)(threadIdx.x >> 6);
    if (blk >= ndilate) return;
    gsr_horizon_dilate(hz.raw, g.tiles_x, g.tiles_y, dilate_r, hz, hz.pyr_out, blk, (int)(threadIdx.x & 63u));
}

#define RW_THREADS 256
__global__ void __launch_bounds__(RW_THREADS)
k_row_work(const uint4* __restrict__ tile_work, const uint4* __restrict__ work_a, GsrSumArgs g, unsigned long long* __restrict__ rows, uint32_t ticket)
{
    const int gty = (int)blockIdx.x * (RW_THREADS / 64) + (int)(threadIdx.x >> 6), lane = (int)(threadIdx.x & 63u);
    if (gty >= g.tiles_y) return;
    unsigned long long sum = 0ull;
    if (gsr_shard_owns(g.shard, gty)) {
        const int base = gsr_shard_local_row(g.shard, gty) * g.tiles_x;
        for (int tx = lane; tx < g.tiles_x; tx += 64) {
            const int i = base + tx;
            if (i >= g.n_tiles) break;
            uint4 w = tile_work[i];
            if (work_a) {
                const uint4 wa = work_a[i];
                if (wa.w & 1u) w = make_uint4(0u, 0u, 0u, 0u);
                sum += gsr_tile_weight(wa);
            }
            sum += gsr_tile_weight(w);
        }
    }
#pragma unroll
    for (int d = 32; d > 0; d >>= 1) sum += __shfl_down(sum, d, 64);
    if (lane == 0) rows[gty] = ((unsigned long long)ticket << 32) | (sum > 0xffffffffull ? 0xffffffffull : sum);
}
```

houdini-gsplat-renderer_amd/engine.py:

```python
from __future__ import annotations

import ctypes as C
import os

import numpy as np

from . import build as _build

_LIB = None


class GsrError(RuntimeError):
    def __init__(self, code: int, msg: str):
        super().__init__(f"gsplat_hip error {code}: {msg}")
        self.code = code


class gsr_camera(C.Structure):
    _fields_ = [("obj_view", C.c_float * 16), ("object", C.c_float * 16), ("inv_object", C.c_float * 16),
                ("view", C.c_float * 16), ("proj", C.c_float * 16), ("cam_pos", C.c_float * 3),
                ("width", C.c_int32), ("height", C.c_int32), ("sh_order", C.c_int32)]


class gsr_stats(C.Structure):
    _fields_ = [("n_splats", C.c_int64), ("n_visible", C.c_int64), ("pairs_total", C.c_int64),
                ("pairs_consumed", C.c_int64), ("tiles_x", C.c_int32), ("tiles_y", C.c_int32),
                ("record_bytes", C.c_int32), ("pair_bytes", C.c_int32),
                ("ms_preprocess", C.c_float), ("ms_depth_sort", C.c_float), ("ms_emit", C.c_float),
                ("ms_tile_sort", C.c_float), ("ms_blend", C.c_float), ("ms_total", C.c_float),
                ("blend_ms_total", C.c_double), ("blend_launches", C.c_int64),
                ("blend_pairs_consumed_total", C.c_int64), ("frame_ms_total", C.c_double), ("frames", C.c_int64),
                ("entries_scanned", C.c_int64), ("blend_entries_scanned_total", C.c_int64),
                ("super_tile", C.c_int32), ("stiles_x", C.c_int32), ("stiles_y", C.c_int32), ("reserved_", C.c_int32),
                ("blend_wave_evals_total", C.c_int64), ("stage_ms_total", C.c_double * 5),
                ("stage_frames", C.c_int64), ("sorts_skipped", C.c_int64), ("frames_requeued", C.c_int64),
                ("lazy_redo_tiles", C.c_int64), ("lazy_colours_total", C.c_int64), ("frames_truncated", C.c_int64),
                ("frames_culled", C.c_int64), ("frames_repaired", C.c_int64),
                ("clusters_total", C.c_int64), ("clusters_kept", C.c_int64),
                ("policy_bits", C.c_int32), ("cull_dilate", C.c_int32), ("cull_holdoff", C.c_int32), ("reserved2_", C.c_int32),
                ("frames_resorted", C.c_int64), ("frames_slab", C.c_int64), ("frames_jumped", C.c_int64), ("frames_lazy", C.c_int64),
                ("uploads", C.c_int64), ("upload_ms", C.c_double * 6),
                ("moves", C.c_int64), ("move_ms", C.c_double * 4)]

    def as_dict(self) -> dict:
        d = {n: getattr(self, n) for n, _ in self._fields_}
        d["stage_ms_total"] = list(self.stage_ms_total)
        d["upload_ms"] = list(self.upload_ms)
        d["move_ms"] = list(self.move_ms)
        return d


class gsr_debug_record(C.Structure):
    _fields_ = [(n, C.c_float) for n in
                ("cx", "cy", "a1x", "a1y", "b1x", "b1y", "hx", "hy", "r", "g", "b", "la", "key")] + \
               [("visible", C.c_int32)]


DEBUG_RECORD_DTYPE = np.dtype([(n, np.float32) for n in
                               ("cx", "cy", "a1x", "a1y", "b1x", "b1y", "hx", "hy", "r", "g", "b", "la", "key")]
                              + [("visible", np.int32)])


class GSplatRenderContext(C.Structure):
    _fields_ = [("obj_view", C.c_float * 16), ("object", C.c_float * 16), ("inv_object", C.c_float * 16),
                ("view", C.c_float * 16), ("proj", C.c_float * 16), ("width", C.c_int32), ("height", C.c_int32),
                ("target", C.c_void_p), ("target_is_device", C.c_int32),
                ("depth", C.c_void_p), ("depth_is_device", C.c_int32)]


class gsr_raw_attrs(C.Structure):
    _fields_ = [("P", C.c_void_p), ("Cd", C.c_void_p), ("alpha", C.c_void_p), ("scale", C.c_void_p), ("orient", C.c_void_p),
                ("sh_scheme", C.c_int32), ("sh_vec3_per_point", C.c_int32), ("sh_array", C.c_void_p), ("sh_ptr", C.POINTER(C.c_void_p))]


class gsr_background(C.Structure):
    _fields_ = [("kind", C.c_int32), ("format", C.c_int32), ("rgba", C.c_float * 4), ("image", C.c_void_p),
                ("image_is_device", C.c_int32), ("reserved_", C.c_int32)]


class gsr_attr_update(C.Structure):
    _fields_ = [("Cd", C.c_void_p), ("alpha", C.c_void_p), ("scale", C.c_void_p), ("orient", C.c_void_p),
                ("shx", C.c_void_p), ("shy", C.c_void_p), ("shz", C.c_void_p)]


class gsr_device_attrs(C.Structure):
    _fields_ = [("P", C.c_void_p), ("Cd", C.c_void_p), ("alpha", C.c_void_p), ("scale", C.c_void_p), ("orient", C.c_void_p),
                ("sh", C.c_void_p), ("sh_vec3_per_point", C.c_int32), ("reserved_", C.c_int32)]


class gsr_read_arrays(C.Structure):
    _fields_ = [("P", C.c_void_p), ("Cd", C.c_void_p), ("alpha", C.c_void_p), ("scale", C.c_void_p), ("orient", C.c_void_p),
                ("shx", C.c_void_p), ("shy", C.c_void_p), ("shz", C.c_void_p)]


class gsr_device_out(C.Structure):
    _fields_ = [("P", C.c_void_p), ("Cd", C.c_void_p), ("alpha", C.c_void_p), ("scale", C.c_void_p), ("orient", C.c_void_p),
                ("sh", C.c_void_p), ("sh_vec3_per_point", C.c_int32), ("reserved_", C.c_int32)]


class gsr_crop_volume(C.Structure):
    _fields_ = [("kind", C.c_int32), ("invert", C.c_int32), ("to_unit", C.c_float * 12)]


class gsr_visibility(C.Structure):
    _fields_ = [("n_volumes", C.c_int32), ("reserved_", C.c_int32), ("volume", gsr_crop_volume * 4),
                ("mask", C.c_void_p), ("mask_splats", C.c_int64)]


class gsplat_attrs(C.Structure):
    _fields_ = [("count", C.c_int64), ("P", C.c_void_p), ("Cd", C.c_void_p), ("opacity", C.c_void_p), ("Alpha", C.c_void_p),
                ("scale", C.c_void_p), ("orient", C.c_void_p), ("sh_coefficients", C.c_void_p),
                ("sh_coefficients_len", C.c_int32), ("sh", C.POINTER(C.c_void_p)), ("f_rest", C.POINTER(C.c_void_p)),
                ("sh_order", C.POINTER(C.c_int32)), ("explicit_camera_pos", C.POINTER(C.c_float))]


TRANSPORT_AUTO, TRANSPORT_RCCL, TRANSPORT_COPY = 0, 1, 2
MAX_DIM = 16384
MISSING_CD, MISSING_OPACITY, MISSING_SCALE, MISSING_ORIENT, MISSING_SH, BAD_SH_ORDER = 1, 2, 4, 8, 16, 32
OPT_XCD_SWIZZLE, OPT_STAGE_TIMING, OPT_SORT_CACHE, OPT_SUPER_TILE, OPT_DEBUG_FLAGS, OPT_FRAMES_IN_FLIGHT, OPT_DEFERRED_CHECK, OPT_LAZY_COLOUR, OPT_SHARD_LAYOUT = 1, 2, 3, 4, 5, 6, 7, 8, 9
OPT_OCCLUSION_CULL = 10
OPT_TIMING_EVERY = 11
OPT_CLUSTER_CULL = 12
OPT_STORAGE_ORDER = 13
OPT_CULL_DILATE = 14
OPT_LOCAL_SORT = 15
OPT_FRONT_SLAB = 16
OPT_ROW_WORK = 17
TILE = 16

TARGET_RGBA32F = 0
TARGET_RGBA16F = 1
TARGET_RGBA8 = 2
AOV_DEPTH = 1
BG_COLOUR = 1
BG_IMAGE = 2
VIS_MAX_VOLUMES = 4
VOL_BOX = 1
VOL_ELLIPSOID = 2
REMOVE_HIDDEN = 1
REMOVE_BLOCK = 4096
TARGET_DTYPES = {TARGET_RGBA32F: np.dtype(np.float32), TARGET_RGBA16F: np.dtype(np.float16), TARGET_RGBA8: np.dtype(np.uint8)}

C_ABI_SYMBOLS = [
    "gsr_device_count", "gsr_create", "gsr_destroy", "gsr_last_error", "gsr_version", "gsr_set_stream",
    "gsr_upload_begin", "gsr_upload_append", "gsr_upload_append_raw", "gsr_upload_end", "gsr_upload_abort", "gsr_upload", "gsr_set_row_shard", "gsr_band_rows",
    "gsr_stitch_bands", "gsr_render", "gsr_render_depth", "gsr_render_wire", "gsr_render_wire_over", "gsr_synchronize", "gsr_get_stats", "gsr_stats_reset", "gsr_set_option",
    "gsr_debug_read_records", "gsr_debug_read_depth_order", "gsr_debug_read_storage_order", "gsr_debug_read_tile_lists", "gsr_debug_sort_pairs", "gsr_debug_sort_pairs_local", "gsr_debug_policy", "gsr_debug_policy_state", "gsr_debug_frame_plan",
    "gsr_debug_read_tile_work", "gsr_debug_read_horizons", "gsr_debug_read_cull",
    "gsr_multi_create", "gsr_multi_destroy", "gsr_multi_count", "gsr_multi_transport", "gsr_multi_context",
    "gsr_multi_set_stream", "gsr_multi_set_option", "gsr_multi_upload_begin", "gsr_multi_upload_append",
    "gsr_multi_upload_end", "gsr_multi_upload_abort", "gsr_multi_upload", "gsr_multi_render", "gsr_multi_render_depth",
    "gsr_multi_synchronize", "gsr_multi_get_stats", "gsr_multi_comm_info", "gsr_multi_gather_stats",
    "gsr_comm_available", "gsr_comm_get_unique_id", "gsr_comm_init", "gsr_comm_info", "gsr_comm_destroy", "gsr_comm_render",
    "gsplat_renderer_create_multi", "gsplat_renderer_multi",
    "gsplat_prim_create", "gsplat_prim_destroy", "gsplat_prim_update", "gsplat_prim_render", "gsplat_prim_missing",
    "gsplat_prim_sh_order", "gsplat_prim_has_sh", "gsplat_prim_array",
    "gsplat_renderer_create", "gsplat_renderer_get_instance", "gsplat_renderer_destroy",
    "gsplat_renderer_register_update", "gsplat_renderer_include_in_render_pass",
    "gsplat_renderer_flush_entries_for_matching_detail", "gsplat_renderer_generate_render_geometry",
    "gsplat_renderer_render", "gsplat_renderer_post_render", "gsplat_renderer_redraw", "gsplat_renderer_set_rendering_enabled",
    "gsplat_renderer_set_explicit_camera_pos", "gsplat_renderer_set_spherical_harmonics_order",
    "gsplat_renderer_query", "gsplat_renderer_get_origin", "gsplat_renderer_get_last_camera_pos",
    "gsplat_renderer_engine", "gsplat_closest_sqrt_power_of_2", "gsplat_quantize_half",
    "gsplat_pack_sh_from_vec3", "gsplat_pack_sh_from_frest", "gsplat_pack_sh_from_array",
    "gsr_target_pixel_bytes", "gsr_set_target_format", "gsr_get_target_format", "gsr_multi_set_target_format", "gsr_convert_pixels",
    "gsplat_renderer_set_target_format", "gsplat_renderer_get_target_format",
    "gsr_render_aov", "gsr_resolve_depth", "gsr_resolve_depth_device", "gsplat_renderer_set_aov_target",
    "gsr_render_over", "gsr_composite_over", "gsplat_renderer_set_background",
    "gsr_update", "gsr_multi_update", "gsr_debug_read_resident", "gsplat_renderer_update_attributes", "gsplat_renderer_row_array",
    "gsr_move", "gsr_multi_move", "gsplat_renderer_move_splats",
    "gsr_upload_append_device", "gsr_update_device", "gsr_move_device", "gsr_debug_check_device_source",
    "gsr_set_row_band", "gsr_read_row_work", "gsr_debug_balance_rows", "gsr_multi_get_bands",
    "gsr_set_visibility", "gsr_get_visibility", "gsr_visibility_eval", "gsr_multi_set_visibility", "gsplat_renderer_set_visibility",
    "gsr_remove", "gsr_remove_map", "gsr_get_removal", "gsr_multi_remove",
    "gsr_add", "gsr_add_device", "gsr_add_capacity", "gsr_get_add", "gsr_multi_add",
    "gsr_read_info", "gsr_read", "gsr_read_device", "gsr_get_read", "gsr_multi_read",
]


def balance_rows(row_work, count: int, cur_first=None, min_gain_permille: int = 0):
    L = load_library()
    w = np.ascontiguousarray(row_work, dtype=np.uint32).reshape(-1)
    cur = None if cur_first is None else np.ascontiguousarray(cur_first, dtype=np.int32).reshape(-1)
    if cur is not None and cur.size != count + 1:
        raise ValueError("cur_first holds count + 1 boundaries")
    out = np.zeros(max(int(count), 0) + 1, np.int32)
    rc = L.gsr_debug_balance_rows(_ptr(w) if w.size else None, int(w.size), int(count), _ptr(cur), int(min_gain_permille), out.ctypes.data)
    _check(rc if rc < 0 else 0)
    return bool(rc), out


POLICY_FIELDS = ("cull_pays", "cull_weak", "vis_unculled", "cull_holdoff", "cull_backoff", "cull_streak", "cull_dilate", "opt_dilate",
                 "slab_holdoff", "local_fails", "local_holdoff")


def lib_path() -> str:
    return os.environ.get("GSR_LIBRARY") or _build.LIB


def load_library() -> C.CDLL:
    global _LIB
    if _LIB is not None:
        return _LIB
    path = lib_path()
    if not os.path.exists(path):
        raise GsrError(-100, f"{path} is missing: run __graft_entry__.build() (hipcc --offload-arch=gfx950) first")
    L = C.CDLL(path)
    vp, i32, i64, f32p = C.c_void_p, C.c_int, C.c_int64, C.POINTER(C.c_float)
    L.gsr_device_count.restype = i32
    L.gsr_last_error.restype = C.c_char_p
    L.gsr_version.restype = C.c_char_p
    L.gsr_create.argtypes = [i32, C.POINTER(vp)]
    L.gsr_destroy.argtypes = [vp]
    L.gsr_destroy.restype = None
    L.gsr_set_stream.argtypes = [vp, vp]
    L.gsr_upload_begin.argtypes = [vp, i64, i32, f32p]
    L.gsr_upload_append.argtypes = [vp, i64] + [vp] * 8
    L.gsr_upload_append_raw.argtypes = [vp, i64, C.POINTER(gsr_raw_attrs)]
    L.gsr_upload_end.argtypes = [vp]
    L.gsr_update.argtypes = [vp, i64, i64, C.POINTER(gsr_attr_update)]
    L.gsr_multi_update.argtypes = [vp, i64, i64, C.POINTER(gsr_attr_update)]
    L.gsr_move.argtypes = [vp, i64, i64, vp, f32p, C.POINTER(gsr_attr_update)]
    L.gsr_multi_move.argtypes = [vp, i64, i64, vp, f32p, C.POINTER(gsr_attr_update)]
    L.gsplat_renderer_move_splats.argtypes = [vp, C.c_char_p, vp, f32p] + [vp] * 7 + [C.POINTER(C.c_int64), C.POINTER(C.c_int64)]
    L.gsr_upload_append_device.argtypes = [vp, i64, C.POINTER(gsr_device_attrs)]
    L.gsr_update_device.argtypes = [vp, i64, i64, C.POINTER(gsr_device_attrs)]
    L.gsr_move_device.argtypes = [vp, i64, i64, f32p, C.POINTER(gsr_device_attrs)]
    L.gsr_debug_check_device_source.argtypes = [vp, vp, i64]
    L.gsr_debug_read_resident.argtypes = [vp, i32, vp, i64]
    L.gsr_set_visibility.argtypes = [vp, C.POINTER(gsr_visibility)]
    L.gsr_get_visibility.argtypes = [vp, C.POINTER(gsr_visibility), C.POINTER(C.c_int64)]
    L.gsr_visibility_eval.argtypes = [C.POINTER(gsr_visibility), vp, i64, i64, vp]
    L.gsr_multi_set_visibility.argtypes = [vp, C.POINTER(gsr_visibility)]
    L.gsplat_renderer_set_visibility.argtypes = [vp, C.POINTER(gsr_visibility)]
    L.gsr_remove.argtypes = [vp, vp, i32, i32, C.POINTER(C.c_int64)]
    L.gsr_remove_map.argtypes = [vp, i64, vp, C.POINTER(C.c_int64)]
    L.gsr_get_removal.argtypes = [vp, C.POINTER(C.c_int64), C.POINTER(C.c_int64), C.POINTER(C.c_double)]
    L.gsr_multi_remove.argtypes = [vp, vp, i32, C.POINTER(C.c_int64)]
    L.gsr_add.argtypes = [vp, i64] + [vp] * 8 + [C.POINTER(C.c_int64)]
    L.gsr_add_device.argtypes = [vp, i64, C.POINTER(gsr_device_attrs), C.POINTER(C.c_int64)]
    L.gsr_add_capacity.argtypes = [i64, i64]
    L.gsr_add_capacity.restype = i64
    L.gsr_get_add.argtypes = [vp] + [C.POINTER(C.c_int64)] * 4 + [C.POINTER(C.c_double)]
    L.gsr_multi_add.argtypes = [vp, i64] + [vp] * 8 + [C.POINTER(C.c_int64)]
    L.gsr_read_info.argtypes = [vp, C.POINTER(C.c_int64), C.POINTER(C.c_int), f32p]
    L.gsr_read.argtypes = [vp, i64, i64, C.POINTER(gsr_read_arrays)]
    L.gsr_read_device.argtypes = [vp, i64, i64, C.POINTER(gsr_device_out)]
    L.gsr_get_read.argtypes = [vp, C.POINTER(C.c_int64), C.POINTER(C.c_int64), C.POINTER(C.c_double)]
    L.gsr_multi_read.argtypes = [vp, i64, i64, C.POINTER(gsr_read_arrays)]
    L.gsplat_renderer_update_attributes.argtypes = [vp, C.c_char_p] + [vp] * 7 + [C.POINTER(C.c_int64), C.POINTER(C.c_int64)]
    L.gsplat_renderer_row_array.argtypes = [vp, C.c_char_p, i32]
    L.gsplat_renderer_row_array.restype = vp
    L.gsr_upload_abort.argtypes = [vp]
    L.gsr_upload.argtypes = [vp, i64] + [vp] * 8 + [f32p]
    L.gsr_set_row_shard.argtypes = [vp, i32, i32]
    L.gsr_band_rows.argtypes = [i32, i32, i32]
    L.gsr_stitch_bands.argtypes = [vp, vp, i32, i32, i32, vp]
    L.gsr_render.argtypes = [vp, C.POINTER(gsr_camera), vp, i32]
    L.gsr_render_depth.argtypes = [vp, C.POINTER(gsr_camera), vp, i32, vp, i32]
    L.gsr_render_aov.argtypes = [vp, C.POINTER(gsr_camera), vp, i32, vp, i32, i32, vp]
    L.gsr_resolve_depth.argtypes = [vp, i64, C.c_float, vp]
    L.gsr_resolve_depth_device.argtypes = [vp, vp, i64, C.c_float, vp]
    L.gsplat_renderer_set_aov_target.argtypes = [vp, i32, vp]
    L.gsr_render_over.argtypes = [vp, C.POINTER(gsr_camera), vp, i32, C.POINTER(gsr_background), vp, i32]
    L.gsr_composite_over.argtypes = [vp, i64, C.POINTER(gsr_background), i32, vp]
    L.gsplat_renderer_set_background.argtypes = [vp, C.POINTER(gsr_background)]
    L.gsr_render_wire.argtypes = [vp, C.POINTER(gsr_camera), vp, i32]
    L.gsr_render_wire_over.argtypes = [vp, C.POINTER(gsr_camera), vp, i32]
    L.gsr_synchronize.argtypes = [vp]
    L.gsr_get_stats.argtypes = [vp, C.POINTER(gsr_stats)]
    L.gsr_stats_reset.argtypes = [vp]
    L.gsr_set_option.argtypes = [vp, i32, i32]
    L.gsr_debug_read_records.argtypes = [vp, vp, i64]
    L.gsr_debug_read_depth_order.argtypes = [vp, vp, i64, C.POINTER(C.c_int64)]
    L.gsr_debug_read_cull.argtypes = [vp, vp, i64, vp, i64, C.POINTER(C.c_int64)]
    L.gsr_debug_read_tile_lists.argtypes = [vp, vp, vp, i64, vp, i64]
    L.gsr_debug_read_storage_order.argtypes = [vp, vp, i64]
    L.gsr_debug_sort_pairs.argtypes = [vp, vp, vp, i64, i32]
    L.gsr_debug_sort_pairs_local.argtypes = [vp, vp, vp, i64, i32, C.c_uint32, i32]
    L.gsr_debug_policy.argtypes = [vp, i32, C.c_longlong, C.c_longlong]
    L.gsr_debug_policy_state.argtypes = [vp, vp]
    L.gsr_debug_frame_plan.argtypes = [i32, vp, vp, vp]
    L.gsr_debug_read_tile_work.argtypes = [vp, vp, i64]
    L.gsr_debug_read_horizons.argtypes = [vp, vp, i64]
    L.gsr_target_pixel_bytes.argtypes = [i32]
    L.gsr_set_target_format.argtypes = [vp, i32]
    L.gsr_get_target_format.argtypes = [vp]
    L.gsr_multi_set_target_format.argtypes = [vp, i32]
    L.gsr_convert_pixels.argtypes = [vp, i64, i32, vp]
    L.gsplat_renderer_set_target_format.argtypes = [vp, i32]
    L.gsplat_renderer_get_target_format.argtypes = [vp]
    L.gsplat_renderer_create.restype = vp
    L.gsplat_renderer_create.argtypes = [i32]
    L.gsplat_renderer_get_instance.restype = vp
    L.gsplat_renderer_destroy.argtypes = [vp]
    L.gsplat_renderer_destroy.restype = None
    L.gsplat_renderer_register_update.argtypes = [vp, C.c_uint64, C.POINTER(C.c_int64), i64, i64, f32p] + [vp] * 8 + \
                                                 [i64, C.c_char_p, i32]
    L.gsplat_renderer_include_in_render_pass.argtypes = [vp, C.c_char_p]
    L.gsplat_renderer_include_in_render_pass.restype = None
    L.gsplat_renderer_flush_entries_for_matching_detail.argtypes = [vp, C.c_char_p]
    L.gsplat_renderer_flush_entries_for_matching_detail.restype = None
    L.gsplat_renderer_generate_render_geometry.argtypes = [vp, C.POINTER(GSplatRenderContext)]
    L.gsplat_renderer_generate_render_geometry.restype = None
    L.gsplat_renderer_render.argtypes = [vp, C.POINTER(GSplatRenderContext), i32]
    L.gsplat_renderer_render.restype = None
    L.gsplat_renderer_post_render.argtypes = [vp]
    L.gsplat_renderer_post_render.restype = None
    L.gsplat_renderer_redraw.argtypes = [vp, C.POINTER(C.c_char_p), i32, C.POINTER(GSplatRenderContext), i32]
    L.gsplat_renderer_redraw.restype = None
    L.gsplat_renderer_set_rendering_enabled.argtypes = [vp, i32]
    L.gsplat_renderer_set_rendering_enabled.restype = None
    L.gsplat_renderer_set_explicit_camera_pos.argtypes = [vp, f32p]
    L.gsplat_renderer_set_explicit_camera_pos.restype = None
    L.gsplat_renderer_set_spherical_harmonics_order.argtypes = [vp, i32]
    L.gsplat_renderer_set_spherical_harmonics_order.restype = None
    L.gsplat_renderer_query.argtypes = [vp, i32, C.c_char_p]
    L.gsplat_renderer_query.restype = i64
    L.gsplat_renderer_get_origin.argtypes = [vp, f32p]
    L.gsplat_renderer_get_origin.restype = None
    L.gsplat_renderer_get_last_camera_pos.argtypes = [vp, f32p]
    L.gsplat_renderer_get_last_camera_pos.restype = None
    L.gsplat_renderer_engine.argtypes = [vp]
    L.gsplat_renderer_engine.restype = vp
    L.gsplat_closest_sqrt_power_of_2.argtypes = [i32]
    L.gsplat_closest_sqrt_power_of_2.restype = C.c_uint
    L.gsplat_quantize_half.argtypes = [vp, vp, i64]
    L.gsplat_quantize_half.restype = None
    L.gsplat_pack_sh_from_vec3.argtypes = [C.POINTER(vp), i64, vp, vp, vp]
    L.gsplat_pack_sh_from_vec3.restype = None
    L.gsplat_pack_sh_from_frest.argtypes = [C.POINTER(vp), i64, vp, vp, vp]
    L.gsplat_pack_sh_from_frest.restype = None
    L.gsplat_pack_sh_from_array.argtypes = [vp, i64, i32, vp, vp, vp]
    L.gsplat_pack_sh_from_array.restype = None
    L.gsr_multi_create.argtypes = [C.POINTER(C.c_int), i32, i32, C.POINTER(vp)]
    L.gsr_multi_destroy.argtypes = [vp]
    L.gsr_multi_destroy.restype = None
    L.gsr_multi_count.argtypes = [vp]
    L.gsr_multi_transport.argtypes = [vp]
    L.gsr_multi_context.argtypes = [vp, i32]
    L.gsr_multi_context.restype = vp
    L.gsr_multi_set_stream.argtypes = [vp, vp]
    L.gsr_multi_set_option.argtypes = [vp, i32, i32]
    L.gsr_multi_upload_begin.argtypes = [vp, i64, i32, f32p]
    L.gsr_multi_upload_append.argtypes = [vp, i64] + [vp] * 8
    L.gsr_multi_upload_end.argtypes = [vp]
    L.gsr_multi_upload_abort.argtypes = [vp]
    L.gsr_multi_upload.argtypes = [vp, i64] + [vp] * 8 + [f32p]
    L.gsr_multi_render.argtypes = [vp, C.POINTER(gsr_camera), vp, i32]
    L.gsr_multi_render_depth.argtypes = [vp, C.POINTER(gsr_camera), vp, i32, vp, i32]
    L.gsr_multi_synchronize.argtypes = [vp]
    L.gsr_multi_get_stats.argtypes = [vp, i32, C.POINTER(gsr_stats)]
    L.gsr_multi_comm_info.argtypes = [vp, C.POINTER(C.c_int), C.POINTER(C.c_int)]
    L.gsr_set_row_band.argtypes = [vp, i32, i32]
    L.gsr_read_row_work.argtypes = [vp, vp, i32, C.POINTER(C.c_int64)]
    L.gsr_debug_balance_rows.argtypes = [vp, i32, i32, vp, i32, vp]
    L.gsr_multi_get_bands.argtypes = [vp, vp, C.POINTER(C.c_int64)]
    L.gsr_multi_gather_stats.argtypes = [vp, i32, C.POINTER(C.c_double), C.POINTER(C.c_int64)]
    L.gsr_comm_info.argtypes = [vp, C.POINTER(C.c_int), C.POINTER(C.c_int)]
    L.gsr_comm_get_unique_id.argtypes = [vp]
    L.gsr_comm_init.argtypes = [vp, vp, i32, i32]
    L.gsr_comm_destroy.argtypes = [vp]
    L.gsr_comm_render.argtypes = [vp, C.POINTER(gsr_camera), vp, i32, vp]
    L.gsplat_renderer_create_multi.argtypes = [C.POINTER(C.c_int), i32, i32]
    L.gsplat_renderer_create_multi.restype = vp
# ... 1106 lines not shown
```

include/gsplat_hip.h:

```cpp
#ifndef GSPLAT_HIP_H
#define GSPLAT_HIP_H

#include <stdint.h>

#ifdef __cplusplus
extern "C" {
#endif

#define GSR_OK                0
#define GSR_E_INVALID        -1
#define GSR_E_HIP            -2
#define GSR_E_NO_DEVICE      -3
#define GSR_E_NO_GEOMETRY    -4
#define GSR_E_TOO_MANY_PAIRS -5
#define GSR_E_OOM            -6
#define GSR_E_COMM           -7

#define GSR_TILE              16
#define GSR_MAX_DIM           16384
#define GSR_MAX_PAIRS         0x7fffff00ll

typedef struct gsr_context gsr_context;

typedef struct gsr_camera {
    float obj_view[16];
    float object[16];
    float inv_object[16];
    float view[16];
    float proj[16];
    float cam_pos[3];
    int32_t width;
    int32_t height;
    int32_t sh_order;
} gsr_camera;

typedef struct gsr_stats {
    int64_t n_splats;
    int64_t n_visible;
    int64_t pairs_total;
    int64_t pairs_consumed;
    int32_t tiles_x, tiles_y;
    int32_t record_bytes;
    int32_t pair_bytes;
    float ms_preprocess, ms_depth_sort, ms_emit, ms_tile_sort, ms_blend, ms_total;
    double blend_ms_total;
    int64_t blend_launches;
    int64_t blend_pairs_consumed_total;
    double frame_ms_total;
    int64_t frames;
    int64_t entries_scanned;
    int64_t blend_entries_scanned_total;
    int32_t super_tile;
    int32_t stiles_x, stiles_y;
    int32_t reserved_;
    int64_t blend_wave_evals_total;
    double stage_ms_total[5];
    int64_t stage_frames;
    int64_t sorts_skipped;
    int64_t frames_requeued;
    int64_t lazy_redo_tiles;
    int64_t lazy_colours_total;
    int64_t frames_truncated;
    int64_t frames_culled;
    int64_t frames_repaired;
    int64_t clusters_total;
    int64_t clusters_kept;
    int32_t policy_bits;
    int32_t cull_dilate;
    int32_t cull_holdoff;
    int32_t reserved2_;
    int64_t frames_resorted;
    int64_t frames_slab;
    int64_t frames_jumped;
    int64_t frames_lazy;
    int64_t uploads;
    double upload_ms[6];
    int64_t moves;
    double move_ms[4];
} gsr_stats;

int  gsr_device_count(void);
int  gsr_create(int device, gsr_context** out);
void gsr_destroy(gsr_context* ctx);
const char* gsr_last_error(void);
const char* gsr_version(void);

int  gsr_set_stream(gsr_context* ctx, void* hip_stream);

#define GSR_TARGET_RGBA32F    0
#define GSR_TARGET_RGBA16F    1
#define GSR_TARGET_RGBA8      2
int  gsr_target_pixel_bytes(int format);
int  gsr_set_target_format(gsr_context* ctx, int format);
int  gsr_get_target_format(gsr_context* ctx);
int  gsr_convert_pixels(const float* rgba32f, int64_t n_pixels, int format, void* out);

int  gsr_upload_begin(gsr_context* ctx, int64_t total_splats, int has_sh, const float origin[3]);
int  gsr_upload_append(gsr_context* ctx, int64_t n,
                       const float* P, const uint16_t* Cd, const float* alpha,
                       const uint16_t* scale, const uint16_t* orient,
                       const uint16_t* shx, const uint16_t* shy, const uint16_t* shz);
typedef struct gsr_raw_attrs {
    const float* P;
    const float* Cd;
    const float* alpha;
    const float* scale;
    const float* orient;
    int32_t sh_scheme;
    int32_t sh_vec3_per_point;
    const float* sh_array;
    const float* const* sh_ptr;
} gsr_raw_attrs;
int  gsr_upload_append_raw(gsr_context* ctx, int64_t n, const gsr_raw_attrs* attrs);
int  gsr_upload_end(gsr_context* ctx);
int  gsr_upload_abort(gsr_context* ctx);
int  gsr_upload(gsr_context* ctx, int64_t n,
                const float* P, const uint16_t* Cd, const float* alpha,
                const uint16_t* scale, const uint16_t* orient,
                const uint16_t* shx, const uint16_t* shy, const uint16_t* shz,
                const float origin[3]);

typedef struct gsr_attr_update {
    const uint16_t* Cd;
    const float*    alpha;
    const uint16_t* scale;
    const uint16_t* orient;
    const uint16_t *shx, *shy, *shz;
} gsr_attr_update;
int  gsr_update(gsr_context* ctx, int64_t first, int64_t n, const gsr_attr_update* u);

int  gsr_move(gsr_context* ctx, int64_t first, int64_t n, const float* P, const float origin[3], const gsr_attr_update* u);

typedef struct gsr_device_attrs {
    const float* P;
    const float* Cd;
    const float* alpha;
    const float* scale;
    const float* orient;
    const float* sh;
    int32_t sh_vec3_per_point;
    int32_t reserved_;
} gsr_device_attrs;
int  gsr_upload_append_device(gsr_context* ctx, int64_t n, const gsr_device_attrs* a);
int  gsr_update_device(gsr_context* ctx, int64_t first, int64_t n, const gsr_device_attrs* a);
int  gsr_move_device(gsr_context* ctx, int64_t first, int64_t n, const float origin[3], const gsr_device_attrs* a);
int  gsr_debug_check_device_source(gsr_context* ctx, const void* p, int64_t bytes);

#define GSR_VIS_MAX_VOLUMES 4
#define GSR_VOL_BOX         1
#define GSR_VOL_ELLIPSOID   2
typedef struct gsr_crop_volume {
    int32_t kind;
    int32_t invert;
// ... 91 lines not shown
#define GSR_COMM_ID_BYTES 128
int  gsr_comm_available(void);
int  gsr_comm_get_unique_id(void* id);
int  gsr_comm_init(gsr_context* ctx, const void* id, int rank, int world);
int  gsr_comm_info(gsr_context* ctx, int* rank, int* nranks);
int  gsr_comm_destroy(gsr_context* ctx);
int  gsr_comm_render(gsr_context* ctx, const gsr_camera* cam, const float* depth, int depth_is_device,
                     float* rgba_out_device);

int  gsr_render(gsr_context* ctx, const gsr_camera* cam, float* rgba_out, int out_is_device);

int  gsr_render_depth(gsr_context* ctx, const gsr_camera* cam, const float* depth, int depth_is_device,
                      float* rgba_out, int out_is_device);

#define GSR_AOV_DEPTH 1
int  gsr_render_aov(gsr_context* ctx, const gsr_camera* cam, const float* depth, int depth_is_device,
                    float* rgba_out, int out_is_device, int aov, float* aov_out);
int  gsr_resolve_depth(const float* aov, int64_t n_pixels, float cov_min, float* depth_out);
int  gsr_resolve_depth_device(gsr_context* ctx, const float* aov, int64_t n_pixels, float cov_min, float* depth_out);

#define GSR_BG_COLOUR 1
#define GSR_BG_IMAGE  2
typedef struct gsr_background {
    int32_t kind;
    int32_t format;
    float   rgba[4];
    const void* image;
    int32_t image_is_device;
    int32_t reserved_;
} gsr_background;
int  gsr_render_over(gsr_context* ctx, const gsr_camera* cam, const float* depth, int depth_is_device,
                     const gsr_background* bg, float* rgba_out, int out_is_device);
int  gsr_composite_over(const float* rgba32f, int64_t n_pixels, const gsr_background* bg,
                        int out_format, void* out);

int  gsr_render_wire(gsr_context* ctx, const gsr_camera* cam, float* rgba_out, int out_is_device);
int  gsr_render_wire_over(gsr_context* ctx, const gsr_camera* cam, float* rgba_inout, int is_device);

int  gsr_synchronize(gsr_context* ctx);
int  gsr_get_stats(gsr_context* ctx, gsr_stats* out);
int  gsr_stats_reset(gsr_context* ctx);

#define GSR_OPT_XCD_SWIZZLE     1
#define GSR_OPT_STAGE_TIMING    2
#define GSR_OPT_SORT_CACHE      3
#define GSR_OPT_SUPER_TILE      4
#define GSR_OPT_FRAMES_IN_FLIGHT 6
#define GSR_OPT_DEBUG_FLAGS     5
#define GSR_OPT_DEFERRED_CHECK   7
#define GSR_OPT_ROW_WORK        17
#define GSR_OPT_SHARD_LAYOUT     9
#define GSR_OPT_TIMING_EVERY    11
#define GSR_OPT_OCCLUSION_CULL  10
#define GSR_OPT_LAZY_COLOUR      8
#define GSR_OPT_CLUSTER_CULL    12
#define GSR_OPT_STORAGE_ORDER   13
#define GSR_OPT_CULL_DILATE     14
#define GSR_OPT_LOCAL_SORT      15
#define GSR_OPT_FRONT_SLAB      16
int  gsr_set_option(gsr_context* ctx, int option, int value);

typedef struct gsr_debug_record {
    float cx, cy, a1x, a1y, b1x, b1y, hx, hy, r, g, b, la;
    float key;
    int32_t visible;
} gsr_debug_record;
int  gsr_debug_read_records(gsr_context* ctx, gsr_debug_record* out, int64_t n);
int  gsr_debug_read_cull(gsr_context* ctx, uint32_t* rect, int64_t n, uint32_t* clusters, int64_t cap, int64_t* n_clusters);
int  gsr_debug_read_depth_order(gsr_context* ctx, int32_t* perm, int64_t cap, int64_t* n_sorted);
int  gsr_debug_read_storage_order(gsr_context* ctx, int32_t* perm, int64_t n);
int  gsr_debug_read_resident(gsr_context* ctx, int which, void* out, int64_t bytes);
int  gsr_debug_read_tile_lists(gsr_context* ctx, int32_t* list_start, int32_t* list_end, int64_t n_lists,
                               int32_t* pair_splat, int64_t n_pairs);

int  gsr_debug_read_tile_work(gsr_context* ctx, uint32_t* work4, int64_t n_tiles);
int  gsr_debug_read_horizons(gsr_context* ctx, float* out4, int64_t n_tiles);

int  gsr_debug_sort_pairs(gsr_context* ctx, uint32_t* keys, uint32_t* vals, int64_t n, int key_bits);
int  gsr_debug_sort_pairs_local(gsr_context* ctx, uint32_t* keys, uint32_t* vals, int64_t n, int key_bits,
                                uint32_t bucket_lo, int bucket_shift);
int  gsr_debug_policy(int32_t* state16, int event, long long a, long long b);
int  gsr_debug_policy_state(gsr_context* ctx, int32_t* state16);
int  gsr_debug_frame_plan(int which, const int32_t* in, int32_t* policy16, int32_t* out);

#ifdef __cplusplus
}
#endif
#endif
```

Measured before the change: 4564.

## Add optional tick-weighted tile ordering and invalidate order table on regime change

Adds an opt-in mode (GSR_ORDER_BY=ticks) in which the blend kernel records per-tile wall-clock ticks and the tile-order builder balances work across XCDs using those measured costs instead of the tile_work weight estimate. The order-table keep/refresh decision moves into a separate plan function that also drops a cached order when the render regime (one-pass, temporal cull, slab) changes. It also adds a specialised k_blend<false> instantiation with an SGPR cap. By default the tick path is off, so the live changes are the regime-aware invalidation, which can trigger extra order rebuilds, and the SGPR-limited kernel variant, which changes register allocation.

```diff
diff --git a/houdini-gsplat-renderer_amd/csrc/gsr_api.hip b/houdini-gsplat-renderer_amd/csrc/gsr_api.hip
--- a/houdini-gsplat-renderer_amd/csrc/gsr_api.hip
+++ b/houdini-gsplat-renderer_amd/csrc/gsr_api.hip
@@ -129,6 +129,7 @@
     size_t pair_cap = 0;
     int32_t *sstart = nullptr, *send = nullptr;
     uint4* tile_work = nullptr;
+    uint32_t* tile_ticks = nullptr;
     size_t tile_cap = 0;
     uint4* tile_work_a = nullptr;
     float* tbuf = nullptr;
@@ -142,6 +143,7 @@
     bool order_valid = false;
     int order_age = 0;
     int order_sig[6] = {0, 0, 0, 0, 0, 0}, order_per_xcd = 0;
+    int order_regime = 0;
     uint32_t* st_scan = nullptr;
     GsrTilePartial* partial = nullptr;
     uint32_t* sup_work = nullptr;
@@ -242,6 +244,7 @@
     uint32_t* blk_pre = nullptr;
     size_t blk_pre_cap = 0;
     int opt_order_keep = 32;
+    int opt_order_by_ticks = 0;
     int opt_fuse_order = 1;
     int opt_mid_sort = 1;
     int opt_host_bands = 4;
@@ -458,7 +461,7 @@
     slot_free_splat_arrays(sl);
     dev_free(sl.hist); dev_free(sl.totals);
     dev_free(sl.pvA);
-    dev_free(sl.sstart); dev_free(sl.send); dev_free(sl.tile_work); dev_free(sl.order); dev_free(sl.sup_work); sl.fb.release(); dev_free(sl.fb32); sl.aovb.release(); sl.bgb.release();
+    dev_free(sl.sstart); dev_free(sl.send); dev_free(sl.tile_work); dev_free(sl.tile_ticks); dev_free(sl.order); dev_free(sl.sup_work); sl.fb.release(); dev_free(sl.fb32); sl.aovb.release(); sl.bgb.release();
     dev_free(sl.hpyr); dev_free(sl.hpyr_next); dev_free(sl.hraw); dev_free(sl.hstat); dev_free(sl.hpyr2); dev_free(sl.slab); dev_free(sl.tile_work_a); dev_free(sl.tbuf); dev_free(sl.ccnt); dev_free(sl.bkt_key); dev_free(sl.bkt_val); dev_free(sl.bkt_cnt); dev_free(sl.d_counts); dev_free(sl.st_scan); dev_free(sl.partial);
     if (sl.h_end) (void)hipHostFree(sl.h_end); if (sl.h_rows) (void)hipHostFree(sl.h_rows); sl.depth_stage.release(); dev_free(sl.dpyr); dev_free(sl.dactive);
     dev_free(sl.redo); dev_free(sl.lazy_ctr); dev_free(sl.colour_evals);
@@ -493,6 +496,7 @@
     if (const char* e = std::getenv("GSR_HOST_BANDS")) c->opt_host_bands = std::min(std::max(std::atoi(e), 1), GSR_HOST_BANDS_MAX);
     if (const char* e = std::getenv("GSR_MID_SORT")) c->opt_mid_sort = std::atoi(e);
     if (const char* e = std::getenv("GSR_FUSE_ORDER")) c->opt_fuse_order = std::atoi(e);
+    if (const char* e = std::getenv("GSR_ORDER_BY")) c->opt_order_by_ticks = std::strcmp(e, "ticks") == 0;
     if (const char* e = std::getenv("GSR_SLAB_FRAC")) { const int v = std::atoi(e); if (v >= 1 && v <= 255) c->slab_frac = v; }
     if (const char* e = std::getenv("GSR_SLAB_MIN")) { const int v = std::atoi(e); if (v >= 1) c->slab_min = v; }
     if (const char* e = std::getenv("GSR_SLAB_MAX")) { const int v = std::atoi(e); if (v >= 1) c->slab_max = v; }
@@ -1508,6 +1512,8 @@
     a.list_cap = list_cap(sl);
     a.sup_work = (a.use_map && c->opt_swizzle >= 2 && sl.sup_work) ? sl.sup_work + 256 * sl.sup_par : nullptr;
     a.slab = j.phase; a.tbuf = sl.tbuf; a.tile_work_a = sl.tile_work_a;
+    a.tile_ticks = sl.tile_ticks;
+    if (c->opt_order_by_ticks && sl.tile_ticks) a.flags |= GSR_BLEND_TICKS;
     uint4* const tw = j.phase == 1 ? sl.tile_work_a : sl.tile_work;
     int sig[6];
     tile_sig(f, sig);
@@ -1615,12 +1621,15 @@
     sl.hstat_valid = hz.raw != nullptr;
     int osig[6];
     tile_sig(j.f, osig);
-    const bool order_due = c->opt_swizzle >= 3 || (c->opt_swizzle == 2 && c->order_pays);
-    const bool order_kept = !order_due && c->opt_swizzle == 2 && c->opt_order_keep > 0 && sl.order_valid && sl.order_age < c->opt_order_keep &&
-                            std::memcmp(osig, sl.order_sig, sizeof osig) == 0;
-    const bool order_refresh = !order_due && !order_kept && c->opt_swizzle == 2 && c->opt_order_keep > 0 && c->n >= 1000000u;
-    if (order_kept) sl.order_age += 1; else sl.order_valid = false;
-    const bool order_now = j.use_map && (order_due || order_refresh) && j.local_tiles > 0 && j.n_super <= 256 && sl.sup_work;
+    GsrOrderIn oi;
+    oi.opt_swizzle = c->opt_swizzle; oi.opt_order_keep = c->opt_order_keep; oi.order_pays = c->order_pays; oi.n = c->n;
+    oi.can_build = j.use_map && j.local_tiles > 0 && j.n_super <= 256 && sl.sup_work;
+    oi.table_valid = sl.order_valid; oi.table_age = sl.order_age; oi.same_shape = std::memcmp(osig, sl.order_sig, sizeof osig) == 0;
+    oi.table_regime = sl.order_regime; oi.regime = gsr_order_regime(j.cull, j.phase);
+    const GsrOrderPlan op = gsr_order_plan(oi);
+    sl.order_valid = op.kept; sl.order_age = op.table_age;
+    const bool order_now = op.build;
+    const uint32_t* const order_ticks = c->opt_order_by_ticks ? sl.tile_ticks : (const uint32_t*)nullptr;
     const int per_xcd = 2 * ((j.n_super + 15) / 16) << (2 * j.f.super_shift);
     if (order_now && (size_t)8 * per_xcd > sl.order_cap) {
         const int rc = regrow(s, sl.order, sl.order_cap, (size_t)8 * per_xcd, (size_t)8 * per_xcd);
@@ -1629,7 +1638,7 @@
     const bool fused_order = order_now && c->opt_fuse_order != 0;
     if (sl.horizon_valid) sl.hpyr_re = std::min(c->cull_pol.dilate, GSR_DILATE_EXACT_MAX);
     if (fused_order) {
-        const GsrOrderArgs oa{sl.tile_work, j.f.tiles_y, sl.sup_work + 256 * sl.sup_par, per_xcd, sl.order};
+        const GsrOrderArgs oa{sl.tile_work, order_ticks, j.f.tiles_y, sl.sup_work + 256 * sl.sup_par, per_xcd, sl.order};
         const int ndil = sl.horizon_valid ? nblocks8 : 0;
         hipLaunchKernelGGL(k_frame_end_order, dim3(9u + (unsigned)((ndil + TO_THREADS / 64 - 1) / (TO_THREADS / 64))), dim3(TO_THREADS), 0, s, sl.partial, nblocks8, ndil, g, sl.counters, sl.d_n, sl.d_frame,
                            prefix_arg, redo_arg, sl.colour_evals, sl.lazy_ctr + 1, sl.sstart, sl.send, c->lazy_hint, work_next, hz, sl.st_scan, sl.hpyr_re, oa);
@@ -1651,7 +1660,7 @@
     }
     if (order_now) {
         if (!fused_order) {
-            hipLaunchKernelGGL(k_tile_order, dim3(8), dim3(TO_THREADS), 0, s, sl.tile_work, g, j.f.tiles_y, sl.sup_work + 256 * sl.sup_par,
+            hipLaunchKernelGGL(k_tile_order, dim3(8), dim3(TO_THREADS), 0, s, sl.tile_work, order_ticks, g, j.f.tiles_y, sl.sup_work + 256 * sl.sup_par,
                                per_xcd, sl.order);
             HIP_TRY(hipGetLastError());
         }
@@ -1659,6 +1668,8 @@
         sl.order_per_xcd = per_xcd;
         sl.order_valid = true;
         sl.order_age = 0;
+        sl.order_regime = op.table_regime;
+        c->st.orders_built += 1;
     }
     if (c->opt_row_work && sl.h_rows_dev) {
         hipLaunchKernelGGL(k_row_work, dim3((unsigned)((j.f.tiles_y + RW_THREADS / 64 - 1) / (RW_THREADS / 64))), dim3(RW_THREADS), 0, s, sl.tile_work,
@@ -2023,10 +2034,11 @@
 
     if ((size_t)j.local_tiles + 1 > sl.tile_cap || !sl.sstart) {
         HIP_TRY(hipStreamSynchronize(s));
-        dev_free(sl.tile_work); dev_free(sl.tile_work_a); dev_free(sl.sstart); dev_free(sl.send); dev_free(sl.redo);
+        dev_free(sl.tile_work); dev_free(sl.tile_ticks); dev_free(sl.tile_work_a); dev_free(sl.sstart); dev_free(sl.send); dev_free(sl.redo);
         sl.tile_cap = 0;
-        if ((rc = dev_alloc(&sl.tile_work, (size_t)j.local_tiles + 1)) || (rc = dev_alloc(&sl.tile_work_a, (size_t)j.local_tiles + 1)) || (rc = dev_alloc(&sl.sstart, (size_t)65536 + 1)) ||
+        if ((rc = dev_alloc(&sl.tile_work, (size_t)j.local_tiles + 1)) || (rc = dev_alloc(&sl.tile_ticks, (size_t)j.local_tiles + 1)) || (rc = dev_alloc(&sl.tile_work_a, (size_t)j.local_tiles + 1)) || (rc = dev_alloc(&sl.sstart, (size_t)65536 + 1)) ||
             (rc = dev_alloc(&sl.send, (size_t)65536 + 1)) || (rc = dev_alloc(&sl.redo, (size_t)j.local_tiles + 1))) return rc;
+        HIP_TRY(hipMemsetAsync(sl.tile_ticks, 0, ((size_t)j.local_tiles + 1) * sizeof(uint32_t), s));
         sl.tile_cap = (size_t)j.local_tiles + 1;
     }
     if (j.phase == 1 && j.out_px > sl.tbuf_cap && (rc = regrow(s, sl.tbuf, sl.tbuf_cap, j.out_px, j.out_px))) return rc;
@@ -2584,6 +2596,12 @@
 {
     if (!in || !out || (which == 0 && !policy16)) return set_err(GSR_E_INVALID, "gsr_debug_frame_plan: NULL argument");
     return gsr_frame_plan_apply(which, in, policy16, out) ? set_err(GSR_E_INVALID, "gsr_debug_frame_plan: unknown selector %d", which) : GSR_OK;
+}
+extern "C" int gsr_debug_order_plan(const int32_t* in, int32_t* out)
+{
+    if (!in || !out) return set_err(GSR_E_INVALID, "gsr_debug_order_plan: NULL argument");
+    gsr_order_plan_apply(in, out);
+    return GSR_OK;
 }
 extern "C" int gsr_debug_policy_state(gsr_context* c, int32_t* state16)
 {
diff --git a/houdini-gsplat-renderer_amd/csrc/gsr_frame_plan.h b/houdini-gsplat-renderer_amd/csrc/gsr_frame_plan.h
--- a/houdini-gsplat-renderer_amd/csrc/gsr_frame_plan.h
+++ b/houdini-gsplat-renderer_amd/csrc/gsr_frame_plan.h
@@ -235,6 +235,52 @@
     return o;
 }
 
+enum GsrOrderRegime : int { GSR_ORDER_ONE_PASS = 0, GSR_ORDER_TEMPORAL = 1, GSR_ORDER_SLAB = 2 };
+static inline int gsr_order_regime(bool cull, int phase) { return phase == 2 ? GSR_ORDER_SLAB : (cull ? GSR_ORDER_TEMPORAL : GSR_ORDER_ONE_PASS); }
+
+#define GSR_ORDER_IN_FIELDS(X)                                                                                                     \
+    X(int, opt_swizzle) X(int, opt_order_keep)                                                                                  \
+    X(bool, order_pays)                                                          \
+    X(uint32_t, n)                                                                                         \
+    X(bool, can_build)                             \
+    X(bool, table_valid) X(int, table_age) X(bool, same_shape) X(int, table_regime)                                             \
+    X(int, regime)
+#define GSR_ORDER_OUT_FIELDS(X)                                                                                                    \
+    X(bool, build)                                                                      \
+    X(bool, kept)                                                                                  \
+    X(bool, table_valid) X(int, table_age) X(int, table_regime)
+
+#define GSR_PLAN_DECLARE(t, name) t name{};
+struct GsrOrderIn { GSR_ORDER_IN_FIELDS(GSR_PLAN_DECLARE) };
+struct GsrOrderPlan { GSR_ORDER_OUT_FIELDS(GSR_PLAN_DECLARE) };
+#undef GSR_PLAN_DECLARE
+
+inline GsrOrderPlan gsr_order_plan(const GsrOrderIn& in)
+{
+    GsrOrderPlan o;
+    const bool due = in.opt_swizzle >= 3 || (in.opt_swizzle == 2 && in.order_pays);
+    o.kept = !due && in.opt_swizzle == 2 && in.opt_order_keep > 0 && in.table_valid && in.table_age < in.opt_order_keep && in.same_shape &&
+             in.table_regime == in.regime;
+    const bool refresh = !due && !o.kept && in.opt_swizzle == 2 && in.opt_order_keep > 0 && in.n >= 1000000u;
+    o.build = in.can_build && (due || refresh);
+    o.table_valid = o.kept || o.build;
+    o.table_age = o.build ? 0 : (o.kept ? in.table_age + 1 : in.table_age);
+    o.table_regime = o.build ? in.regime : in.table_regime;
+    return o;
+}
+inline void gsr_order_plan_apply(const int32_t* in, int32_t* out)
+{
+    int k = 0, o = 0;
+    GsrOrderIn v;
+#define GSR_GET(t, name) v.name = (t)(uint32_t)in[k++];
+#define GSR_PUT(t, name) out[o++] = (int32_t)r.name;
+    GSR_ORDER_IN_FIELDS(GSR_GET)
+    const GsrOrderPlan r = gsr_order_plan(v);
+    GSR_ORDER_OUT_FIELDS(GSR_PUT)
+#undef GSR_GET
+#undef GSR_PUT
+}
+
 #define GSR_PLAN_HINT_FIELDS(X) X(uint32_t, surv_hint) X(uint32_t, kept_hint) X(uint32_t, kept_lo) X(uint32_t, kept_hi) X(bool, kept_culled) \
     X(uint32_t, slab_kept) X(uint32_t, slab_kept1) X(uint32_t, slab_kept2)
 inline int gsr_frame_plan_apply(int which, const int32_t* in, int32_t* policy, int32_t* out)
diff --git a/houdini-gsplat-renderer_amd/csrc/k_blend.h b/houdini-gsplat-renderer_amd/csrc/k_blend.h
--- a/houdini-gsplat-renderer_amd/csrc/k_blend.h
+++ b/houdini-gsplat-renderer_amd/csrc/k_blend.h
@@ -62,7 +62,10 @@
     int32_t row_lo, row_hi;
     int32_t out_format;
     void* out_packed;
+    uint32_t* tile_ticks;
 };
+#define GSR_BLEND_TICKS 0x40000000
+__device__ __forceinline__ uint32_t gsr_add_sat(uint32_t a, uint32_t b) { const uint32_t s = a + b; return s < a ? 0xffffffffu : s; }
 
 #if BL_WAVES_PER_EU > 0
 #define BL_OCC __attribute__((amdgpu_waves_per_eu(BL_WAVES_PER_EU)))
@@ -101,6 +104,7 @@
     __shared__ uint32_t slastu[4];
     __shared__ uint32_t stail[32];
     __shared__ uint32_t slast[4];
+    __shared__ uint32_t sticks0;
 
     int tile;
     if (LAZY) {
@@ -137,6 +141,15 @@
     const float tcx0 = (float)(tx * GSR_TILE_PX) + 0.5f, tcy0 = (float)(gty * GSR_TILE_PX) + 0.5f;
     const float qcx = tcx0 + 3.5f + 8.0f * (float)(wave & 1), qcy = tcy0 + 3.5f + 8.0f * (float)(wave >> 1);
     if (tid == 0) { sevals = 0; sredo = 0; sdmet = 0; }
+    const uint32_t ticks_in = (a.flags & GSR_BLEND_TICKS) ? (uint32_t)wall_clock64() : 0u;
+    auto leave_ticks = [&](int t, uint32_t now) __attribute__((always_inline)) -> uint32_t {
+        uint32_t d = now - sticks0;
+        d = d ? d : 1u;
+        uint32_t* const tt = a.tile_ticks;
+        if (LAZY || a.slab == 2) { const uint32_t tot = gsr_add_sat(tt[t], d); tt[t] = tot; return LAZY ? tot : d; }
+        tt[t] = d;
+        return d;
+    };
     if (tid < 4) slast[tid] = 0u;
     uint32_t my_evals = 0;
     uint32_t my_last = 0;
@@ -151,6 +164,7 @@
     const int e_ = send[st] < a.list_cap ? send[st] : a.list_cap;
     const int n = e_ > s ? e_ - s : 0;
     if (!HAS_DEPTH && a.guard && (guard_now != 0u) != (a.guard_want != 0u)) return;
+    if (tid == 0 && (a.flags & GSR_BLEND_TICKS)) sticks0 = ticks_in;
 
     gsr_v2f C01 = {0.0f, 0.0f};
     float C2 = 0.0f, T = 1.0f;
@@ -454,6 +468,7 @@
             int t3 = tile;
             asm volatile("" : "+s"(t3));
             if (tid == 0 && lz.redo) lz.redo[atomicAdd(lz.redo_count, 1u)] = t3;
+            if (tid == 0 && (a.flags & GSR_BLEND_TICKS)) (void)leave_ticks(t3, (uint32_t)wall_clock64());
             return;
         }
         if (HAS_DEPTH && zfilter) {
@@ -467,6 +482,7 @@
         }
         if ((dall & 1u) != 0u) { saturated = true; break; }
     }
+    const uint32_t ticks_out = (a.flags & GSR_BLEND_TICKS) ? (uint32_t)wall_clock64() : 0u;
     if (pix_ok) {
         int t2 = tid;
         asm volatile("" : "+v"(t2));
@@ -498,7 +514,7 @@
         unsigned long long* o = g_blend_prof[blockIdx.x][wave];
 #pragma unroll
         for (int i = 0; i < 9; ++i) o[i] = prof[i];
-        o[9] = 1ull; o[10] = (unsigned long long)round; o[11] = wall0; o[12] = wall_clock64();
+        o[9] = 1ull | ((unsigned long long)(uint32_t)tile << 32); o[10] = (unsigned long long)round; o[11] = wall0; o[12] = wall_clock64();
         o[13] = occ_lanes; o[14] = occ_evals; o[15] = occ_half | (occ_none << 32);
     }
 #endif
@@ -517,7 +533,9 @@
         const uint32_t fs = (uint32_t)(first_hit_step < 0 ? 0 : (first_hit_step > 0x1fff ? 0x1fff : first_hit_step)) | (sdmet ? 0x2000u : 0u);
         const uint4 tw = make_uint4((uint32_t)(rd < n ? rd : n), fetched, sevals, (saturated ? 1u : 0u) | (fs << 1) | (u_all ? 0x8000u : 0u) | (es_c << 16) | (es_u << 24));
         tile_work[tile] = tw;
-        if (a.sup_work && gsr_tile_weight(tw)) atomicAdd(&a.sup_work[st], gsr_tile_weight(tw));
+        const uint32_t ticks = (a.flags & GSR_BLEND_TICKS) ? leave_ticks(tile, ticks_out) : 0u;
+        const uint32_t sw = (a.flags & GSR_BLEND_TICKS) ? ticks : gsr_tile_weight(tw);
+        if (a.sup_work && sw) atomicAdd(&a.sup_work[st], sw);
     }
 }
 
@@ -529,6 +547,15 @@
         const float* __restrict__ zwin, const float* __restrict__ depth, GsrLazyArgs lz)
 {
     gsr_blend_tile<HAS_DEPTH, false>(a, tile_map, svals, sstart, send, recs, out, tile_work, zwin, depth, lz);
+}
+template <>
+__global__ void __launch_bounds__(256) BL_OCC __attribute__((amdgpu_num_sgpr(96)))
+k_blend<false>(GsrBlendArgs a, const int32_t* __restrict__ tile_map, const uint2* __restrict__ svals,
+               const int32_t* __restrict__ sstart, const int32_t* __restrict__ send,
+               const GsrRecord* __restrict__ recs, float4* __restrict__ out, uint4* __restrict__ tile_work,
+               const float* __restrict__ zwin, const float* __restrict__ depth, GsrLazyArgs lz)
+{
+    gsr_blend_tile<false, false>(a, tile_map, svals, sstart, send, recs, out, tile_work, zwin, depth, lz);
 }
 template <bool HAS_DEPTH>
 __global__ void __launch_bounds__(256)
@@ -951,8 +978,8 @@
 #define TO_THREADS 1024
 #define TO_LEVELS 128
 __device__ __forceinline__ void
-gsr_tile_order(const uint4* __restrict__ tile_work, const GsrSumArgs& g, int tiles_y, const uint32_t* __restrict__ sup_work, int cap,
-               int32_t* __restrict__ order, const int xcd)
+gsr_tile_order(const uint4* __restrict__ tile_work, const uint32_t* __restrict__ tile_ticks , const GsrSumArgs& g, int tiles_y,
+               const uint32_t* __restrict__ sup_work, int cap, int32_t* __restrict__ order, const int xcd)
 {
     __shared__ uint32_t s_sup[256];
     __shared__ uint32_t s_own[64];
@@ -989,7 +1016,7 @@
         const int lty = gsr_shard_local_row(g.shard, gty);
         const int i = lty * g.tiles_x + tx;
         if (i >= g.n_tiles) return -1;
-        w = gsr_tile_weight(tile_work[i]);
+        w = tile_ticks ? tile_ticks[i] : gsr_tile_weight(tile_work[i]);
         return i;
     };
     constexpr int TO_CACHE = 5;
@@ -1043,13 +1070,13 @@
     for (int p = (int)s_nown + tid; p < cap; p += TO_THREADS) order[8 * p + xcd] = -1;
 }
 __global__ void __launch_bounds__(TO_THREADS)
-k_tile_order(const uint4* __restrict__ tile_work, GsrSumArgs g, int tiles_y, const uint32_t* __restrict__ sup_work, int cap,
-             int32_t* __restrict__ order)
-{
-    gsr_tile_order(tile_work, g, tiles_y, sup_work, cap, order, (int)blockIdx.x);
-}
-
-struct GsrOrderArgs { const uint4* tile_work; int32_t tiles_y; const uint32_t* sup_work; int32_t cap; int32_t* order; };
+k_tile_order(const uint4* __restrict__ tile_work, const uint32_t* __restrict__ tile_ticks, GsrSumArgs g, int tiles_y,
+             const uint32_t* __restrict__ sup_work, int cap, int32_t* __restrict__ order)
+{
+    gsr_tile_order(tile_work, tile_ticks, g, tiles_y, sup_work, cap, order, (int)blockIdx.x);
+}
+
+struct GsrOrderArgs { const uint4* tile_work; const uint32_t* tile_ticks; int32_t tiles_y; const uint32_t* sup_work; int32_t cap; int32_t* order; };
 __global__ void __launch_bounds__(TO_THREADS)
 k_frame_end_order(const GsrTilePartial* __restrict__ partial, int nblocks, int ndilate , GsrSumArgs g,
                   unsigned long long* __restrict__ counters, const uint32_t* __restrict__ n_visible, unsigned long long* __restrict__ summary,
@@ -1060,7 +1087,7 @@
 {
     const int b = (int)blockIdx.x;
     if (b < 8) {
-        gsr_tile_order(oa.tile_work, g, oa.tiles_y, oa.sup_work, oa.cap, oa.order, b);
+        gsr_tile_order(oa.tile_work, oa.tile_ticks, g, oa.tiles_y, oa.sup_work, oa.cap, oa.order, b);
         return;
     }
     if (b == 8) {
diff --git a/houdini-gsplat-renderer_amd/engine.py b/houdini-gsplat-renderer_amd/engine.py
--- a/houdini-gsplat-renderer_amd/engine.py
+++ b/houdini-gsplat-renderer_amd/engine.py
@@ -37,7 +37,7 @@
                 ("lazy_redo_tiles", C.c_int64), ("lazy_colours_total", C.c_int64), ("frames_truncated", C.c_int64),
                 ("frames_culled", C.c_int64), ("frames_repaired", C.c_int64),
                 ("clusters_total", C.c_int64), ("clusters_kept", C.c_int64),
-                ("policy_bits", C.c_int32), ("cull_dilate", C.c_int32), ("cull_holdoff", C.c_int32), ("reserved2_", C.c_int32),
+                ("policy_bits", C.c_int32), ("cull_dilate", C.c_int32), ("cull_holdoff", C.c_int32), ("orders_built", C.c_int32),
                 ("frames_resorted", C.c_int64), ("frames_slab", C.c_int64), ("frames_jumped", C.c_int64), ("frames_lazy", C.c_int64),
                 ("uploads", C.c_int64), ("upload_ms", C.c_double * 6),
                 ("moves", C.c_int64), ("move_ms", C.c_double * 4)]
@@ -145,7 +145,7 @@
     "gsr_device_count", "gsr_create", "gsr_destroy", "gsr_last_error", "gsr_version", "gsr_set_stream",
     "gsr_upload_begin", "gsr_upload_append", "gsr_upload_append_raw", "gsr_upload_end", "gsr_upload_abort", "gsr_upload", "gsr_set_row_shard", "gsr_band_rows",
     "gsr_stitch_bands", "gsr_render", "gsr_render_depth", "gsr_render_wire", "gsr_render_wire_over", "gsr_synchronize", "gsr_get_stats", "gsr_stats_reset", "gsr_set_option",
-    "gsr_debug_read_records", "gsr_debug_read_depth_order", "gsr_debug_read_storage_order", "gsr_debug_read_tile_lists", "gsr_debug_sort_pairs", "gsr_debug_sort_pairs_local", "gsr_debug_policy", "gsr_debug_policy_state", "gsr_debug_frame_plan",
+    "gsr_debug_read_records", "gsr_debug_read_depth_order", "gsr_debug_read_storage_order", "gsr_debug_read_tile_lists", "gsr_debug_sort_pairs", "gsr_debug_sort_pairs_local", "gsr_debug_policy", "gsr_debug_policy_state", "gsr_debug_frame_plan", "gsr_debug_order_plan",
     "gsr_debug_read_tile_work", "gsr_debug_read_horizons", "gsr_debug_read_cull",
     "gsr_multi_create", "gsr_multi_destroy", "gsr_multi_count", "gsr_multi_transport", "gsr_multi_context",
     "gsr_multi_set_stream", "gsr_multi_set_option", "gsr_multi_upload_begin", "gsr_multi_upload_append",
@@ -281,6 +281,7 @@
     L.gsr_debug_policy.argtypes = [vp, i32, C.c_longlong, C.c_longlong]
     L.gsr_debug_policy_state.argtypes = [vp, vp]
     L.gsr_debug_frame_plan.argtypes = [i32, vp, vp, vp]
+    L.gsr_debug_order_plan.argtypes = [vp, vp]
     L.gsr_debug_read_tile_work.argtypes = [vp, vp, i64]
     L.gsr_debug_read_horizons.argtypes = [vp, vp, i64]
     L.gsr_target_pixel_bytes.argtypes = [i32]
diff --git a/include/gsplat_hip.h b/include/gsplat_hip.h
--- a/include/gsplat_hip.h
+++ b/include/gsplat_hip.h
@@ -68,7 +68,7 @@
     int32_t policy_bits;
     int32_t cull_dilate;
     int32_t cull_holdoff;
-    int32_t reserved2_;
+    int32_t orders_built;
     int64_t frames_resorted;
     int64_t frames_slab;
     int64_t frames_jumped;
@@ -326,6 +326,7 @@
 int  gsr_debug_policy(int32_t* state16, int event, long long a, long long b);
 int  gsr_debug_policy_state(gsr_context* ctx, int32_t* state16);
 int  gsr_debug_frame_plan(int which, const int32_t* in, int32_t* policy16, int32_t* out);
+int  gsr_debug_order_plan(const int32_t* in, int32_t* out);
 
 #ifdef __cplusplus
 }
```

Result: no change. 4536 (-0.6%).
